# jhbastek/PhysicsInformedDiffusionModels

Hardware: AMD Instinct MI355X
Metric: training samples/sec (UNet+PDE-residual step), 64x64 Darcy (higher is better)
Workload: dtype f32

## Files before the change

### physicsinformeddiffusionmodels_amd/csrc/k_attn_proj.hip

```cpp
#include "pidm_launch.h"

namespace pidm {

static const int kLapDH = 32;
constexpr int kLapSmallNT = 1024;
static const int kLapTileLd = 33;

__device__ __forceinline__ float lap_exp(float x) { return __expf(x); }
__device__ __forceinline__ int lap_row(int r, int half) { return (r & 3) + 8 * (r >> 2) + 4 * half; }

static int lap_nper_div() {
  const char* e = knob("PIDM_LAP_NPER_DIV");
  const int v = e ? atoi(e) : 1;
  return (v == 2 || v == 4) ? v : 1;
}
static int lap_nper(int N, int C, int slabs) {
  int n = (slabs == 1 ? 512 : 256) * 32 / C;
  if (slabs == 3) n = (C == 32) ? 32 : n / 2;
  if (slabs == 2 && n / lap_nper_div() >= 64) n /= lap_nper_div();
  while (n > 32 && N % n) n >>= 1;
  return n;
}

template <int CB>
__global__ void __launch_bounds__(512) lap_kctx_kernel(const float* __restrict__ xn, const float* __restrict__ wqkv,
                                                       float* __restrict__ part, int N, int heads, int nper) {
  constexpr int C = 32 * CB, CP = C + 4;
  HIP_DYNAMIC_SHARED(float, smem)
  float* xs = smem;
  float* fs = smem + (size_t)nper * CP;
  const int tid = threadIdx.x, lane = tid & 63, half = lane >> 5, l31 = lane & 31;
  const int wave = __builtin_amdgcn_readfirstlane(tid >> 6);
  const int NS = N / nper;
  const int b = blockIdx.x / NS, ns = blockIdx.x % NS;
  const int HD = heads * kLapDH;
  const float* xb = xn + ((size_t)b * N + (size_t)ns * nper) * C;
  for (int e = tid; e < nper * (C / 4); e += 512) {
    const int px = e / (C / 4), q = e - px * (C / 4);
    *reinterpret_cast<f32x4*>(xs + (size_t)px * CP + 4 * q) = *reinterpret_cast<const f32x4*>(xb + (size_t)px * C + 4 * q);
  }
  __syncthreads();
  const int h = wave;
  if (h >= heads) return;
  f32x4 wk[C / 8];
  const float* wrow = wqkv + ((size_t)HD + h * kLapDH + l31) * C + 4 * half;
#pragma unroll
  for (int g8 = 0; g8 < C / 8; ++g8) wk[g8] = *reinterpret_cast<const f32x4*>(wrow + 8 * g8);
  f32x16 M[CB];
#pragma unroll
  for (int cb = 0; cb < CB; ++cb)
    for (int r = 0; r < 16; ++r) M[cb][r] = 0.f;
  float mrun = -3.0e38f, zp = 0.f;
  float* fw = fs + wave * 32;
  for (int t = 0; t < nper / 32; ++t) {
    f32x16 kt;
    for (int r = 0; r < 16; ++r) kt[r] = 0.f;
    const float* arow = xs + (size_t)(t * 32 + l31) * CP + 4 * half;
#pragma unroll
    for (int g8 = 0; g8 < C / 8; ++g8) {
      const f32x4 a4 = *reinterpret_cast<const f32x4*>(arow + 8 * g8);
#pragma unroll
      for (int s = 0; s < 4; ++s) kt = __builtin_amdgcn_mfma_f32_32x32x2f32(a4[s], wk[g8][s], kt, 0, 0, 0);
    }
    float tm = kt[0];
#pragma unroll
    for (int r = 1; r < 16; ++r) tm = fmaxf(tm, kt[r]);
    tm = fmaxf(tm, pidm_other_half(tm));
    if (__any(tm > mrun)) {
      const float mn = fmaxf(mrun, tm);
      const float f = lap_exp(mrun - mn);
      zp *= f;
      mrun = mn;
      if (half == 0) fw[l31] = f;
      PIDM_WAVE_LDS_SYNC();
#pragma unroll
      for (int q4 = 0; q4 < 4; ++q4) {
        const f32x4 f4 = *reinterpret_cast<const f32x4*>(fw + 8 * q4 + 4 * half);
#pragma unroll
        for (int cb = 0; cb < CB; ++cb)
#pragma unroll
          for (int i = 0; i < 4; ++i) M[cb][4 * q4 + i] *= f4[i];
      }
      PIDM_WAVE_LDS_SYNC();
    }
#pragma unroll
    for (int r = 0; r < 16; ++r) {
      kt[r] = lap_exp(kt[r] - mrun);
      zp += kt[r];
    }
#pragma unroll
    for (int r = 0; r < 16; ++r) {
      const float* brow = xs + (size_t)(t * 32 + lap_row(r, half)) * CP + l31;
#pragma unroll
      for (int cb = 0; cb < CB; ++cb) M[cb] = __builtin_amdgcn_mfma_f32_32x32x2f32(kt[r], brow[32 * cb], M[cb], 0, 0, 0);
    }
  }
  const float z = zp + pidm_other_half(zp);
  float* o = part + ((size_t)blockIdx.x * heads + h) * (size_t)(32 * C + 64);
#pragma unroll
  for (int cb = 0; cb < CB; ++cb)
#pragma unroll
    for (int r = 0; r < 16; ++r) o[(size_t)lap_row(r, half) * C + 32 * cb + l31] = M[cb][r];
  if (half == 0) {
    o[32 * C + l31] = mrun;
    o[32 * C + 32 + l31] = z;
  }
}

static int lap_nper_split(int N, int C) {
  int n = 256 * 32 / C;
  if (n / lap_nper_div() >= 64) n /= lap_nper_div();
  while (n > 32 && N % n) n >>= 1;
  return n;
}
static int lap_groups(int heads, int ntiles) {
  const char* e = knob("PIDM_LAP_GROUPS");
  int g = 8 / heads;
  if (e && atoi(e) > 0 && atoi(e) < g) g = atoi(e);
  while (g > 1 && ntiles % g) --g;
  return g < 1 ? 1 : g;
}
template <int CB>
__global__ void __launch_bounds__(512) lap_kctx_split_kernel(const float* __restrict__ xn, const float* __restrict__ wqkv,
                                                             float* __restrict__ part, int N, int heads, int nper) {
  constexpr int C = 32 * CB, RA = 6 * C + 16;
  HIP_DYNAMIC_SHARED(float, smemf)
  char* smem = reinterpret_cast<char*>(smemf);
  const int RT = nper * 2 + 16;
  char* XA = smem;
  char* XT = smem + (size_t)nper * RA;
  float* fs = reinterpret_cast<float*>(XT + (size_t)3 * C * RT);
  const int tid = threadIdx.x, lane = tid & 63, half = lane >> 5, l31 = lane & 31;
  const int wave = __builtin_amdgcn_readfirstlane(tid >> 6);
  const int NS = N / nper;
  const int b = blockIdx.x / NS, ns = blockIdx.x % NS;
  const int HD = heads * kLapDH;
  const float* xb = xn + ((size_t)b * N + (size_t)ns * nper) * C;
  {
    constexpr int QN = C / 4, GP = 16 / QN;
    const int q = lane & (QN - 1), pb = (lane & 15) / QN, la = lane >> 4;
    for (int sl = wave; sl < nper / (4 * GP); sl += 8) {
      const int px = (sl * GP + pb) * 4 + la;
      const f32x4 v = *reinterpret_cast<const f32x4*>(xb + (size_t)px * C + 4 * q);
      typedef unsigned u32x2_t __attribute__((ext_vector_type(2)));
      unsigned a0, a1, a2, b0, b1, b2;
      pidm_split3_pk(v[0], v[1], a0, a1, a2);
      pidm_split3_pk(v[2], v[3], b0, b1, b2);
      char* da = XA + (size_t)px * RA + 8 * q;
      *reinterpret_cast<u32x2_t*>(da) = u32x2_t{a0, b0};
      *reinterpret_cast<u32x2_t*>(da + 2 * C) = u32x2_t{a1, b1};
      *reinterpret_cast<u32x2_t*>(da + 4 * C) = u32x2_t{a2, b2};
      unsigned t0 = __float_as_uint(v[0]), t1 = __float_as_uint(v[1]), t2 = __float_as_uint(v[2]), t3 = __float_as_uint(v[3]);
      {
        const auto s02 = __builtin_amdgcn_permlane32_swap(t0, t2, false, false);
        const auto s13 = __builtin_amdgcn_permlane32_swap(t1, t3, false, false);
        const auto s01 = __builtin_amdgcn_permlane16_swap(s02[0], s13[0], false, false);
        const auto s23 = __builtin_amdgcn_permlane16_swap(s02[1], s13[1], false, false);
        t0 = s01[0]; t1 = s01[1]; t2 = s23[0]; t3 = s23[1];
      }
      pidm_split3_pk(__uint_as_float(t0), __uint_as_float(t1), a0, a1, a2);
      pidm_split3_pk(__uint_as_float(t2), __uint_as_float(t3), b0, b1, b2);
      char* dt = XT + (size_t)(4 * q + la) * RT + (size_t)((sl * GP + pb) * 4) * 2;
      *reinterpret_cast<u32x2_t*>(dt) = u32x2_t{a0, b0};
      *reinterpret_cast<u32x2_t*>(dt + (size_t)C * RT) = u32x2_t{a1, b1};
      *reinterpret_cast<u32x2_t*>(dt + (size_t)2 * C * RT) = u32x2_t{a2, b2};
    }
  }
  __syncthreads();
  const int h = wave;
  if (h >= heads) return;
  u32x4 wk[C / 16][3];
  {
    const float* wrow = wqkv + ((size_t)HD + h * kLapDH + l31) * C + 8 * half;
#pragma unroll
    for (int s = 0; s < C / 16; ++s) {
      const f32x4 w0 = *reinterpret_cast<const f32x4*>(wrow + 16 * s), w1 = *reinterpret_cast<const f32x4*>(wrow + 16 * s + 4);
      unsigned p0[4], p1[4], p2[4];
      pidm_split3_pk(w0[0], w0[1], p0[0], p1[0], p2[0]);
      pidm_split3_pk(w0[2], w0[3], p0[1], p1[1], p2[1]);
      pidm_split3_pk(w1[0], w1[1], p0[2], p1[2], p2[2]);
      pidm_split3_pk(w1[2], w1[3], p0[3], p1[3], p2[3]);
      wk[s][0] = u32x4{p0[0], p0[1], p0[2], p0[3]};
      wk[s][1] = u32x4{p1[0], p1[1], p1[2], p1[3]};
      wk[s][2] = u32x4{p2[0], p2[1], p2[2], p2[3]};
    }
  }
  f32x16 M[CB];
#pragma unroll
  for (int cb = 0; cb < CB; ++cb)
    for (int r = 0; r < 16; ++r) M[cb][r] = 0.f;
  float mrun = -3.0e38f, zp = 0.f;
  float* fw = fs + wave * 32;
#define PIDM_LAP_SIX(acc_, a_, b_)                                                                                 \
  acc_ = pidm_mfma_bf16_32x32x16(a_[2], b_[0], acc_);                                                              \
  acc_ = pidm_mfma_bf16_32x32x16(a_[0], b_[2], acc_);                                                              \
  acc_ = pidm_mfma_bf16_32x32x16(a_[1], b_[1], acc_);                                                              \
  acc_ = pidm_mfma_bf16_32x32x16(a_[1], b_[0], acc_);                                                              \
  acc_ = pidm_mfma_bf16_32x32x16(a_[0], b_[1], acc_);                                                              \
  acc_ = pidm_mfma_bf16_32x32x16(a_[0], b_[0], acc_);
  for (int t = 0; t < nper / 32; ++t) {
    f32x16 kt;
    for (int r = 0; r < 16; ++r) kt[r] = 0.f;
    const char* arow = XA + (size_t)(t * 32 + l31) * RA + 16 * half;
#pragma unroll
    for (int s = 0; s < C / 16; ++s) {
      u32x4 xa[3];
#pragma unroll
      for (int pc = 0; pc < 3; ++pc) xa[pc] = *reinterpret_cast<const u32x4*>(arow + pc * 2 * C + 32 * s);
      PIDM_LAP_SIX(kt, xa, wk[s])
    }
    float tm = kt[0];
#pragma unroll
    for (int r = 1; r < 16; ++r) tm = fmaxf(tm, kt[r]);
    tm = fmaxf(tm, pidm_other_half(tm));
    if (__any(tm > mrun)) {
      const float mn = fmaxf(mrun, tm);
      const float f = lap_exp(mrun - mn);
      zp *= f;
      mrun = mn;
      if (half == 0) fw[l31] = f;
      PIDM_WAVE_LDS_SYNC();
#pragma unroll
      for (int q4 = 0; q4 < 4; ++q4) {
        const f32x4 f4 = *reinterpret_cast<const f32x4*>(fw + 8 * q4 + 4 * half);
#pragma unroll
        for (int cb = 0; cb < CB; ++cb)
#pragma unroll
          for (int i = 0; i < 4; ++i) M[cb][4 * q4 + i] *= f4[i];
      }
      PIDM_WAVE_LDS_SYNC();
    }
#pragma unroll
    for (int r = 0; r < 16; ++r) {
      kt[r] = lap_exp(kt[r] - mrun);
      zp += kt[r];
    }
#pragma unroll
    for (int s = 0; s < 2; ++s) {
      u32x4 ea[3];
      {
        unsigned p0[4], p1[4], p2[4];
#pragma unroll
        for (int j = 0; j < 4; ++j) pidm_split3_pk(kt[8 * s + 2 * j], kt[8 * s + 2 * j + 1], p0[j], p1[j], p2[j]);
        ea[0] = u32x4{p0[0], p0[1], p0[2], p0[3]};
        ea[1] = u32x4{p1[0], p1[1], p1[2], p1[3]};
        ea[2] = u32x4{p2[0], p2[1], p2[2], p2[3]};
      }
#pragma unroll
      for (int cb = 0; cb < CB; ++cb) {
        u32x4 xb4[3];
        const char* brow = XT + (size_t)(32 * cb + l31) * RT + (size_t)(t * 32 + 16 * s + 4 * half) * 2;
#pragma unroll
        for (int pc = 0; pc < 3; ++pc) {
          typedef unsigned u32x2_t __attribute__((ext_vector_type(2)));
          const u32x2_t lo = *reinterpret_cast<const u32x2_t*>(brow + (size_t)pc * C * RT);
          const u32x2_t hi = *reinterpret_cast<const u32x2_t*>(brow + (size_t)pc * C * RT + 16);
          xb4[pc] = u32x4{lo[0], lo[1], hi[0], hi[1]};
        }
        PIDM_LAP_SIX(M[cb], ea, xb4)
      }
    }
  }
#undef PIDM_LAP_SIX
  const float z = zp + pidm_other_half(zp);
  float* o = part + ((size_t)blockIdx.x * heads + h) * (size_t)(32 * C + 64);
#pragma unroll
  for (int cb = 0; cb < CB; ++cb)
#pragma unroll
    for (int r = 0; r < 16; ++r) o[(size_t)lap_row(r, half) * C + 32 * cb + l31] = M[cb][r];
  if (half == 0) {
    o[32 * C + l31] = mrun;
    o[32 * C + 32 + l31] = z;
  }
}

__global__ void __launch_bounds__(kLapSmallNT) lap_kctx_final_kernel(const float* __restrict__ part, const float* __restrict__ wqkv,
                                                             const float* __restrict__ wout, float* __restrict__ kst,
                                                             float* __restrict__ Mmat, float* __restrict__ ctx,
                                                             float* __restrict__ P, int N, int heads, int C, int NS) {
  HIP_DYNAMIC_SHARED(float, smem)
  float* sM = smem;
  float* sW = sM + 32 * C;
  float* sC = sW + 32 * (C + 1) + C;
  float* sw = sC + 32 * 33;
  float* sst = sw + NS * 32;
  __shared__ float sm_[32], siz[32];
  constexpr int NT = kLapSmallNT;
  const int b = blockIdx.x / heads, h = blockIdx.x % heads, tid = threadIdx.x;
  const int HD = heads * kLapDH;
  const size_t pstride = (size_t)(32 * C + 64);
  const float* p0 = part + ((size_t)b * NS * heads + h) * pstride;
  for (int e = tid; e < NS * 64; e += NT) sst[e] = p0[(size_t)(e >> 6) * heads * pstride + 32 * C + (e & 63)];
  __syncthreads();
  if (tid < 32) {
    float m = -3.0e38f;
    for (int k = 0; k < NS; ++k) m = fmaxf(m, sst[k * 64 + tid]);
    float z = 0.f;
    for (int k = 0; k < NS; ++k) {
      const float w = lap_exp(sst[k * 64 + tid] - m);
      sw[k * 32 + tid] = w;
      z += sst[k * 64 + 32 + tid] * w;
    }
    sm_[tid] = m;
    siz[tid] = 1.f / z;
    kst[((size_t)blockIdx.x * 32 + tid) * 2] = m;
    kst[((size_t)blockIdx.x * 32 + tid) * 2 + 1] = 1.f / z;
  }
  __syncthreads();
  for (int e = tid; e < 32 * C; e += NT) {
    const int d = e / C;
    float v = 0.f;
    for (int k = 0; k < NS; ++k) v += p0[(size_t)k * heads * pstride + e] * sw[k * 32 + d];
    v *= siz[d];
    sM[e] = v;
    Mmat[(size_t)blockIdx.x * 32 * C + e] = v;
    const int c = e - d * C;
    sW[d * (C + 1) + c] = wqkv[((size_t)2 * HD + h * kLapDH + d) * C + c];
  }
  __syncthreads();
  const float invN = 1.f / (float)N;
  for (int e = tid; e < 1024; e += NT) {
    const int d = e >> 5, ee = e & 31;
    float v = 0.f;
    for (int c = 0; c < C; ++c) v = fmaf(sM[d * C + c], sW[ee * (C + 1) + c], v);
    v *= invN;
    sC[d * 33 + ee] = v;
    ctx[(size_t)blockIdx.x * 1024 + e] = v;
  }
  __syncthreads();
  for (int e = tid; e < 32 * C; e += NT) {
    const int cc = e >> 5, ee = e & 31;
    sW[cc * 33 + ee] = wout[(size_t)cc * HD + h * kLapDH + ee];
  }
  __syncthreads();
  for (int e = tid; e < 32 * C; e += NT) {
    const int d = e / C, cc = e - d * C;
    float v = 0.f;
#pragma unroll
    for (int ee = 0; ee < 32; ++ee) v = fmaf(sC[d * 33 + ee], sW[cc * 33 + ee], v);
    P[(size_t)blockIdx.x * 32 * C + e] = v;
  }
}

template <int CB>
__global__ void __launch_bounds__(256) lap_out_kernel(const float* __restrict__ xn, const float* __restrict__ wqkv,
                                                      const float* __restrict__ P, const float* __restrict__ bias,
                                                      const float* __restrict__ resid, float* __restrict__ y,
                                                      float* __restrict__ qstat, int N, int heads, int tiles_per_wg, float scale) {
  constexpr int C = 32 * CB, CP = C + 4;
  HIP_DYNAMIC_SHARED(float, smem)
  const int HD = heads * kLapDH;
  float* sWq = smem;
  float* sP = smem + (size_t)HD * CP;
  const int tid = threadIdx.x, lane = tid & 63, half = lane >> 5, l31 = lane & 31;
  const int wave = __builtin_amdgcn_readfirstlane(tid >> 6);
  const int wgs_per_img = (N / 32 + tiles_per_wg - 1) / tiles_per_wg;
  const int b = blockIdx.x / wgs_per_img, wg = blockIdx.x % wgs_per_img;
  for (int e = tid; e < HD * (C / 4); e += 256) {
    const int row = e / (C / 4), q = e - row * (C / 4);
    *reinterpret_cast<f32x4*>(sWq + (size_t)row * CP + 4 * q) = *reinterpret_cast<const f32x4*>(wqkv + (size_t)row * C + 4 * q);
    *reinterpret_cast<f32x4*>(sP + (size_t)row * C + 4 * q) = *reinterpret_cast<const f32x4*>(P + ((size_t)b * HD + row) * C + 4 * q);
  }
  __syncthreads();
  const int t_end = (wg + 1) * tiles_per_wg < N / 32 ? (wg + 1) * tiles_per_wg : N / 32;
  for (int t = wg * tiles_per_wg + wave; t < t_end; t += 4) {
    const size_t pix = (size_t)b * N + (size_t)t * 32 + l31;
    f32x4 xt[C / 8];
#pragma unroll
    for (int g8 = 0; g8 < C / 8; ++g8) xt[g8] = *reinterpret_cast<const f32x4*>(xn + pix * C + 8 * g8 + 4 * half);
    f32x16 yacc[CB];
#pragma unroll
    for (int cb = 0; cb < CB; ++cb)
      for (int r = 0; r < 16; ++r) yacc[cb][r] = 0.f;
    for (int h = 0; h < heads; ++h) {
      f32x16 qt;
      for (int r = 0; r < 16; ++r) qt[r] = 0.f;
      const float* wrow = sWq + (size_t)(h * kLapDH + l31) * CP + 4 * half;
#pragma unroll
      for (int g8 = 0; g8 < C / 8; ++g8) {
        const f32x4 w4 = *reinterpret_cast<const f32x4*>(wrow + 8 * g8);
#pragma unroll
        for (int s = 0; s < 4; ++s) qt = __builtin_amdgcn_mfma_f32_32x32x2f32(w4[s], xt[g8][s], qt, 0, 0, 0);
      }
      float mx = qt[0];
#pragma unroll
      for (int r = 1; r < 16; ++r) mx = fmaxf(mx, qt[r]);
      mx = fmaxf(mx, pidm_other_half(mx));
      float sm = 0.f;
#pragma unroll
      for (int r = 0; r < 16; ++r) {
        qt[r] = lap_exp(qt[r] - mx);
        sm += qt[r];
      }
      sm += pidm_other_half(sm);
      const float inv = 1.f / sm;
      if (half == 0) *reinterpret_cast<float2*>(qstat + (pix * heads + h) * 2) = make_float2(mx, inv);
      const float sc = inv * scale;
      const float* prow = sP + (size_t)(h * kLapDH) * C + l31;
#pragma unroll
      for (int r = 0; r < 16; ++r) {
        const float qv = qt[r] * sc;
        const float* pr = prow + (size_t)lap_row(r, half) * C;
#pragma unroll
        for (int cb = 0; cb < CB; ++cb) yacc[cb] = __builtin_amdgcn_mfma_f32_32x32x2f32(pr[32 * cb], qv, yacc[cb], 0, 0, 0);
      }
    }
#pragma unroll
    for (int cb = 0; cb < CB; ++cb)
#pragma unroll
      for (int q4 = 0; q4 < 4; ++q4) {
        const int c0 = 32 * cb + 8 * q4 + 4 * half;
        const f32x4 bv = *reinterpret_cast<const f32x4*>(bias + c0);
        const f32x4 rv = *reinterpret_cast<const f32x4*>(resid + pix * C + c0);
        f32x4 o;
#pragma unroll
        for (int i = 0; i < 4; ++i) o[i] = yacc[cb][4 * q4 + i] + bv[i] + rv[i];
        *reinterpret_cast<f32x4*>(y + pix * C + c0) = o;
      }
  }
}

__global__ void __launch_bounds__(512) lap_out_split_kernel(const float* __restrict__ xn, const float* __restrict__ wqkv,
                                                            const float* __restrict__ P, const float* __restrict__ bias,
                                                            const float* __restrict__ resid, float* __restrict__ y,
                                                            float* __restrict__ qstat, int N, int heads, int tiles_per_wg, float scale) {
  constexpr int C = 32, RA = 6 * C + 16;
  HIP_DYNAMIC_SHARED(float, smemf)
  char* smem = reinterpret_cast<char*>(smemf);
  const int HD = heads * kLapDH;
  const int RT = HD * 2 + 16;
  char* WA = smem;
  char* PT = smem + (size_t)HD * RA;
  const int tid = threadIdx.x, lane = tid & 63, half = lane >> 5, l31 = lane & 31;
  const int wave = __builtin_amdgcn_readfirstlane(tid >> 6);
  const int wgs_per_img = (N / 32 + tiles_per_wg - 1) / tiles_per_wg;
  const int b = blockIdx.x / wgs_per_img, wg = blockIdx.x % wgs_per_img;
  typedef unsigned u32x2_t __attribute__((ext_vector_type(2)));
  {
    const int q = lane & 7, pb = (lane >> 3) & 1, la = lane >> 4;
    for (int sl = wave; sl < HD / 8; sl += 8) {
      const int d = (sl * 2 + pb) * 4 + la;
      const f32x4 v = *reinterpret_cast<const f32x4*>(wqkv + (size_t)d * C + 4 * q);
      const f32x4 w = *reinterpret_cast<const f32x4*>(P + ((size_t)b * HD + d) * C + 4 * q);
      unsigned a0, a1, a2, b0, b1, b2;
      pidm_split3_pk(v[0], v[1], a0, a1, a2);
      pidm_split3_pk(v[2], v[3], b0, b1, b2);
      char* da = WA + (size_t)d * RA + 8 * q;
      *reinterpret_cast<u32x2_t*>(da) = u32x2_t{a0, b0};
      *reinterpret_cast<u32x2_t*>(da + 2 * C) = u32x2_t{a1, b1};
      *reinterpret_cast<u32x2_t*>(da + 4 * C) = u32x2_t{a2, b2};
      unsigned t0 = __float_as_uint(w[0]), t1 = __float_as_uint(w[1]), t2 = __float_as_uint(w[2]), t3 = __float_as_uint(w[3]);
      {
        const auto s02 = __builtin_amdgcn_permlane32_swap(t0, t2, false, false);
        const auto s13 = __builtin_amdgcn_permlane32_swap(t1, t3, false, false);
        const auto s01 = __builtin_amdgcn_permlane16_swap(s02[0], s13[0], false, false);
        const auto s23 = __builtin_amdgcn_permlane16_swap(s02[1], s13[1], false, false);
        t0 = s01[0]; t1 = s01[1]; t2 = s23[0]; t3 = s23[1];
      }
      pidm_split3_pk(__uint_as_float(t0), __uint_as_float(t1), a0, a1, a2);
      pidm_split3_pk(__uint_as_float(t2), __uint_as_float(t3), b0, b1, b2);
      char* dt = PT + (size_t)(4 * q + la) * RT + (size_t)((sl * 2 + pb) * 4) * 2;
      *reinterpret_cast<u32x2_t*>(dt) = u32x2_t{a0, b0};
      *reinterpret_cast<u32x2_t*>(dt + (size_t)C * RT) = u32x2_t{a1, b1};
      *reinterpret_cast<u32x2_t*>(dt + (size_t)2 * C * RT) = u32x2_t{a2, b2};
    }
  }
  __syncthreads();
#define PIDM_LAP_SIX(acc_, a_, b_)                                                                                 \
  acc_ = pidm_mfma_bf16_32x32x16(a_[2], b_[0], acc_);                                                              \
  acc_ = pidm_mfma_bf16_32x32x16(a_[0], b_[2], acc_);                                                              \
  acc_ = pidm_mfma_bf16_32x32x16(a_[1], b_[1], acc_);                                                              \
  acc_ = pidm_mfma_bf16_32x32x16(a_[1], b_[0], acc_);                                                              \
  acc_ = pidm_mfma_bf16_32x32x16(a_[0], b_[1], acc_);                                                              \
  acc_ = pidm_mfma_bf16_32x32x16(a_[0], b_[0], acc_);
  const int t_end = (wg + 1) * tiles_per_wg < N / 32 ? (wg + 1) * tiles_per_wg : N / 32;
  for (int t = wg * tiles_per_wg + wave; t < t_end; t += 8) {
    const size_t pix = (size_t)b * N + (size_t)t * 32 + l31;
    u32x4 xb[C / 16][3];
#pragma unroll
    for (int s = 0; s < C / 16; ++s) {
      const f32x4 x0 = *reinterpret_cast<const f32x4*>(xn + pix * C + 16 * s + 8 * half);
      const f32x4 x1 = *reinterpret_cast<const f32x4*>(xn + pix * C + 16 * s + 8 * half + 4);
      unsigned p0[4], p1[4], p2[4];
      pidm_split3_pk(x0[0], x0[1], p0[0], p1[0], p2[0]);
      pidm_split3_pk(x0[2], x0[3], p0[1], p1[1], p2[1]);
      pidm_split3_pk(x1[0], x1[1], p0[2], p1[2], p2[2]);
      pidm_split3_pk(x1[2], x1[3], p0[3], p1[3], p2[3]);
      xb[s][0] = u32x4{p0[0], p0[1], p0[2], p0[3]};
      xb[s][1] = u32x4{p1[0], p1[1], p1[2], p1[3]};
      xb[s][2] = u32x4{p2[0], p2[1], p2[2], p2[3]};
    }
    f32x16 yacc;
    for (int r = 0; r < 16; ++r) yacc[r] = 0.f;
    for (int h = 0; h < heads; ++h) {
      f32x16 qt;
      for (int r = 0; r < 16; ++r) qt[r] = 0.f;
      const char* wrow = WA + (size_t)(h * kLapDH + l31) * RA + 16 * half;
#pragma unroll
      for (int s = 0; s < C / 16; ++s) {
        u32x4 wa[3];
#pragma unroll
        for (int pc = 0; pc < 3; ++pc) wa[pc] = *reinterpret_cast<const u32x4*>(wrow + pc * 2 * C + 32 * s);
        PIDM_LAP_SIX(qt, wa, xb[s])
      }
      float mx = qt[0];
#pragma unroll
      for (int r = 1; r < 16; ++r) mx = fmaxf(mx, qt[r]);
      mx = fmaxf(mx, pidm_other_half(mx));
      float sm = 0.f;
#pragma unroll
      for (int r = 0; r < 16; ++r) {
        qt[r] = lap_exp(qt[r] - mx);
        sm += qt[r];
      }
      sm += pidm_other_half(sm);
      const float inv = 1.f / sm;
      if (half == 0) *reinterpret_cast<float2*>(qstat + (pix * heads + h) * 2) = make_float2(mx, inv);
      const float sc = inv * scale;
#pragma unroll
      for (int s = 0; s < 2; ++s) {
        u32x4 qb[3], pa[3];
        {
          unsigned p0[4], p1[4], p2[4];
#pragma unroll
          for (int j = 0; j < 4; ++j) pidm_split3_pk(qt[8 * s + 2 * j] * sc, qt[8 * s + 2 * j + 1] * sc, p0[j], p1[j], p2[j]);
          qb[0] = u32x4{p0[0], p0[1], p0[2], p0[3]};
          qb[1] = u32x4{p1[0], p1[1], p1[2], p1[3]};
          qb[2] = u32x4{p2[0], p2[1], p2[2], p2[3]};
        }
        const char* prow = PT + (size_t)l31 * RT + (size_t)(h * kLapDH + 16 * s + 4 * half) * 2;
#pragma unroll
        for (int pc = 0; pc < 3; ++pc) {
          const u32x2_t lo = *reinterpret_cast<const u32x2_t*>(prow + (size_t)pc * C * RT);
          const u32x2_t hi = *reinterpret_cast<const u32x2_t*>(prow + (size_t)pc * C * RT + 16);
          pa[pc] = u32x4{lo[0], lo[1], hi[0], hi[1]};
        }
        PIDM_LAP_SIX(yacc, pa, qb)
      }
    }
#pragma unroll
    for (int q4 = 0; q4 < 4; ++q4) {
      const int c0 = 8 * q4 + 4 * half;
      const f32x4 bv = *reinterpret_cast<const f32x4*>(bias + c0);
      const f32x4 rv = *reinterpret_cast<const f32x4*>(resid + pix * C + c0);
      f32x4 o;
#pragma unroll
      for (int i = 0; i < 4; ++i) o[i] = yacc[4 * q4 + i] + bv[i] + rv[i];
      *reinterpret_cast<f32x4*>(y + pix * C + c0) = o;
    }
  }
#undef PIDM_LAP_SIX
}

template <int CB>
__global__ void __launch_bounds__(512) lap_g_kernel(const float* __restrict__ xn, const float* __restrict__ dy,
                                                    const float* __restrict__ wqkv, const float* __restrict__ qstat,
                                                    float* __restrict__ part, int N, int heads, int nper, float scale) {
  constexpr int C = 32 * CB, CP = C + 4;
  HIP_DYNAMIC_SHARED(float, smem)
  float* xs = smem;
  float* ys = smem + (size_t)nper * CP;
  const int tid = threadIdx.x, lane = tid & 63, half = lane >> 5, l31 = lane & 31;
  const int wave = __builtin_amdgcn_readfirstlane(tid >> 6);
  const int NS = N / nper;
  const int b = blockIdx.x / NS, ns = blockIdx.x % NS;
  const size_t pix0 = (size_t)b * N + (size_t)ns * nper;
  for (int e = tid; e < nper * (C / 4); e += 512) {
    const int px = e / (C / 4), q = e - px * (C / 4);
    *reinterpret_cast<f32x4*>(xs + (size_t)px * CP + 4 * q) = *reinterpret_cast<const f32x4*>(xn + (pix0 + px) * C + 4 * q);
    *reinterpret_cast<f32x4*>(ys + (size_t)px * CP + 4 * q) = *reinterpret_cast<const f32x4*>(dy + (pix0 + px) * C + 4 * q);
  }
  __syncthreads();
  const int h = wave;
  if (h >= heads) return;
  f32x4 wq[C / 8];
  const float* wrow = wqkv + ((size_t)h * kLapDH + l31) * C + 4 * half;
#pragma unroll
  for (int g8 = 0; g8 < C / 8; ++g8) wq[g8] = *reinterpret_cast<const f32x4*>(wrow + 8 * g8);
  f32x16 G[CB];
#pragma unroll
  for (int cb = 0; cb < CB; ++cb)
    for (int r = 0; r < 16; ++r) G[cb][r] = 0.f;
  for (int t = 0; t < nper / 32; ++t) {
    f32x16 qt;
    for (int r = 0; r < 16; ++r) qt[r] = 0.f;
    const float* arow = xs + (size_t)(t * 32 + l31) * CP + 4 * half;
#pragma unroll
    for (int g8 = 0; g8 < C / 8; ++g8) {
      const f32x4 a4 = *reinterpret_cast<const f32x4*>(arow + 8 * g8);
#pragma unroll
      for (int s = 0; s < 4; ++s) qt = __builtin_amdgcn_mfma_f32_32x32x2f32(a4[s], wq[g8][s], qt, 0, 0, 0);
    }
    const float* st = qstat + ((pix0 + (size_t)t * 32) * heads + h) * 2;
#pragma unroll
    for (int r = 0; r < 16; ++r) {
      const int px = lap_row(r, half);
      const float2 s2 = *reinterpret_cast<const float2*>(st + (size_t)px * heads * 2);
      const float qv = lap_exp(qt[r] - s2.x) * s2.y * scale;
      const float* brow = ys + (size_t)(t * 32 + px) * CP + l31;
#pragma unroll
      for (int cb = 0; cb < CB; ++cb) G[cb] = __builtin_amdgcn_mfma_f32_32x32x2f32(qv, brow[32 * cb], G[cb], 0, 0, 0);
    }
  }
  float* o = part + ((size_t)blockIdx.x * heads + h) * (size_t)(32 * C);
#pragma unroll
  for (int cb = 0; cb < CB; ++cb)
#pragma unroll
    for (int r = 0; r < 16; ++r) o[(size_t)lap_row(r, half) * C + 32 * cb + l31] = G[cb][r];
}

template <int CB>
__global__ void __launch_bounds__(512) lap_g_split_kernel(const float* __restrict__ xn, const float* __restrict__ dy,
                                                          const float* __restrict__ wqkv, const float* __restrict__ qstat,
                                                          float* __restrict__ part, int N, int heads, int nper, float scale) {
  constexpr int C = 32 * CB, RA = 6 * C + 16;
  HIP_DYNAMIC_SHARED(float, smemf)
  char* smem = reinterpret_cast<char*>(smemf);
  const int RT = nper * 2 + 16;
  char* XA = smem;
  char* YT = smem + (size_t)nper * RA;
  const int tid = threadIdx.x, lane = tid & 63, half = lane >> 5, l31 = lane & 31;
  const int wave = __builtin_amdgcn_readfirstlane(tid >> 6);
  const int NS = N / nper;
  const int b = blockIdx.x / NS, ns = blockIdx.x % NS;
  const size_t pix0 = (size_t)b * N + (size_t)ns * nper;
  {
    constexpr int QN = C / 4, GP = 16 / QN;
    const int q = lane & (QN - 1), pb = (lane & 15) / QN, la = lane >> 4;
    typedef unsigned u32x2_t __attribute__((ext_vector_type(2)));
    for (int sl = wave; sl < nper / (4 * GP); sl += 8) {
      const int px = (sl * GP + pb) * 4 + la;
      const f32x4 v = *reinterpret_cast<const f32x4*>(xn + (pix0 + px) * C + 4 * q);
      const f32x4 w = *reinterpret_cast<const f32x4*>(dy + (pix0 + px) * C + 4 * q);
      unsigned a0, a1, a2, b0, b1, b2;
      pidm_split3_pk(v[0], v[1], a0, a1, a2);
      pidm_split3_pk(v[2], v[3], b0, b1, b2);
      char* da = XA + (size_t)px * RA + 8 * q;
      *reinterpret_cast<u32x2_t*>(da) = u32x2_t{a0, b0};
      *reinterpret_cast<u32x2_t*>(da + 2 * C) = u32x2_t{a1, b1};
      *reinterpret_cast<u32x2_t*>(da + 4 * C) = u32x2_t{a2, b2};
      unsigned t0 = __float_as_uint(w[0]), t1 = __float_as_uint(w[1]), t2 = __float_as_uint(w[2]), t3 = __float_as_uint(w[3]);
      {
        const auto s02 = __builtin_amdgcn_permlane32_swap(t0, t2, false, false);
        const auto s13 = __builtin_amdgcn_permlane32_swap(t1, t3, false, false);
        const auto s01 = __builtin_amdgcn_permlane16_swap(s02[0], s13[0], false, false);
        const auto s23 = __builtin_amdgcn_permlane16_swap(s02[1], s13[1], false, false);
        t0 = s01[0]; t1 = s01[1]; t2 = s23[0]; t3 = s23[1];
      }
      pidm_split3_pk(__uint_as_float(t0), __uint_as_float(t1), a0, a1, a2);
      pidm_split3_pk(__uint_as_float(t2), __uint_as_float(t3), b0, b1, b2);
      char* dt = YT + (size_t)(4 * q + la) * RT + (size_t)((sl * GP + pb) * 4) * 2;
      *reinterpret_cast<u32x2_t*>(dt) = u32x2_t{a0, b0};
      *reinterpret_cast<u32x2_t*>(dt + (size_t)C * RT) = u32x2_t{a1, b1};
      *reinterpret_cast<u32x2_t*>(dt + (size_t)2 * C * RT) = u32x2_t{a2, b2};
    }
  }
  __syncthreads();
  const int h = wave;
  if (h >= heads) return;
  u32x4 wq[C / 16][3];
  {
    const float* wrow = wqkv + ((size_t)h * kLapDH + l31) * C + 8 * half;
#pragma unroll
    for (int s = 0; s < C / 16; ++s) {
      const f32x4 w0 = *reinterpret_cast<const f32x4*>(wrow + 16 * s), w1 = *reinterpret_cast<const f32x4*>(wrow + 16 * s + 4);
      unsigned p0[4], p1[4], p2[4];
      pidm_split3_pk(w0[0], w0[1], p0[0], p1[0], p2[0]);
      pidm_split3_pk(w0[2], w0[3], p0[1], p1[1], p2[1]);
      pidm_split3_pk(w1[0], w1[1], p0[2], p1[2], p2[2]);
      pidm_split3_pk(w1[2], w1[3], p0[3], p1[3], p2[3]);
      wq[s][0] = u32x4{p0[0], p0[1], p0[2], p0[3]};
      wq[s][1] = u32x4{p1[0], p1[1], p1[2], p1[3]};
      wq[s][2] = u32x4{p2[0], p2[1], p2[2], p2[3]};
    }
  }
  f32x16 G[CB];
#pragma unroll
  for (int cb = 0; cb < CB; ++cb)
    for (int r = 0; r < 16; ++r) G[cb][r] = 0.f;
#define PIDM_LAP_SIX(acc_, a_, b_)                                                                                 \
  acc_ = pidm_mfma_bf16_32x32x16(a_[2], b_[0], acc_);                                                              \
  acc_ = pidm_mfma_bf16_32x32x16(a_[0], b_[2], acc_);                                                              \
  acc_ = pidm_mfma_bf16_32x32x16(a_[1], b_[1], acc_);                                                              \
  acc_ = pidm_mfma_bf16_32x32x16(a_[1], b_[0], acc_);                                                              \
  acc_ = pidm_mfma_bf16_32x32x16(a_[0], b_[1], acc_);                                                              \
  acc_ = pidm_mfma_bf16_32x32x16(a_[0], b_[0], acc_);
  for (int t = 0; t < nper / 32; ++t) {
    f32x16 qt;
    for (int r = 0; r < 16; ++r) qt[r] = 0.f;
    const char* arow = XA + (size_t)(t * 32 + l31) * RA + 16 * half;
#pragma unroll
    for (int s = 0; s < C / 16; ++s) {
      u32x4 xa[3];
#pragma unroll
      for (int pc = 0; pc < 3; ++pc) xa[pc] = *reinterpret_cast<const u32x4*>(arow + pc * 2 * C + 32 * s);
      PIDM_LAP_SIX(qt, xa, wq[s])
    }
    const float* st = qstat + ((pix0 + (size_t)t * 32) * heads + h) * 2;
#pragma unroll
    for (int r = 0; r < 16; ++r) {
      const float2 s2 = *reinterpret_cast<const float2*>(st + (size_t)lap_row(r, half) * heads * 2);
      qt[r] = lap_exp(qt[r] - s2.x) * s2.y * scale;
    }
#pragma unroll
    for (int s = 0; s < 2; ++s) {
      u32x4 ea[3];
      {
        unsigned p0[4], p1[4], p2[4];
#pragma unroll
        for (int j = 0; j < 4; ++j) pidm_split3_pk(qt[8 * s + 2 * j], qt[8 * s + 2 * j + 1], p0[j], p1[j], p2[j]);
        ea[0] = u32x4{p0[0], p0[1], p0[2], p0[3]};
        ea[1] = u32x4{p1[0], p1[1], p1[2], p1[3]};
        ea[2] = u32x4{p2[0], p2[1], p2[2], p2[3]};
      }
#pragma unroll
      for (int cb = 0; cb < CB; ++cb) {
        u32x4 yb4[3];
        const char* brow = YT + (size_t)(32 * cb + l31) * RT + (size_t)(t * 32 + 16 * s + 4 * half) * 2;
#pragma unroll
        for (int pc = 0; pc < 3; ++pc) {
          typedef unsigned u32x2_t __attribute__((ext_vector_type(2)));
          const u32x2_t lo = *reinterpret_cast<const u32x2_t*>(brow + (size_t)pc * C * RT);
          const u32x2_t hi = *reinterpret_cast<const u32x2_t*>(brow + (size_t)pc * C * RT + 16);
          yb4[pc] = u32x4{lo[0], lo[1], hi[0], hi[1]};
        }
        PIDM_LAP_SIX(G[cb], ea, yb4)
      }
    }
  }
#undef PIDM_LAP_SIX
  float* o = part + ((size_t)blockIdx.x * heads + h) * (size_t)(32 * C);
#pragma unroll
  for (int cb = 0; cb < CB; ++cb)
#pragma unroll
    for (int r = 0; r < 16; ++r) o[(size_t)lap_row(r, half) * C + 32 * cb + l31] = G[cb][r];
}

__global__ void __launch_bounds__(kLapSmallNT) lap_mid_kernel(const float* __restrict__ gpart, const float* __restrict__ wqkv,
                                                      const float* __restrict__ wout, const float* __restrict__ ctx,
                                                      const float* __restrict__ Mmat, float* __restrict__ dMmat,
                                                      float* __restrict__ rowdot, float* __restrict__ dwout_part,
                                                      float* __restrict__ dwv_part, int N, int heads, int C, int NS) {
  HIP_DYNAMIC_SHARED(float, smem)
  float* sG = smem;
  float* sW = sG + 32 * (C + 1);
  float* sD = sW + (C > 33 ? C : 33) * 33 + 32 * (C + 1);
  float* sM = sD + 32 * 33;
  constexpr int NT = kLapSmallNT;
  const int b = blockIdx.x / heads, h = blockIdx.x % heads, tid = threadIdx.x;
  const int HD = heads * kLapDH;
  const float* g0 = gpart + ((size_t)b * NS * heads + h) * (size_t)(32 * C);
  for (int e = tid; e < 32 * C; e += NT) {
    const int d = e / C, c = e - d * C;
    float v = 0.f;
    for (int k0 = 0; k0 < NS; k0 += 8) {
      float t[8];
#pragma unroll
      for (int u = 0; u < 8; ++u) t[u] = g0[(size_t)(k0 + u < NS ? k0 + u : 0) * heads * 32 * C + e];
#pragma unroll
      for (int u = 0; u < 8; ++u) v += (k0 + u < NS) ? t[u] : 0.f;
    }
    sG[d * (C + 1) + c] = v;
    sM[d * (C + 1) + c] = Mmat[(size_t)blockIdx.x * 32 * C + e];
    const int cc = e >> 5, ee = e & 31;
    sW[cc * 33 + ee] = wout[(size_t)cc * HD + h * kLapDH + ee];
  }
  __syncthreads();
  for (int e = tid; e < 1024; e += NT) {
    const int d = e >> 5, ee = e & 31;
    float v = 0.f;
    for (int c = 0; c < C; ++c) v = fmaf(sG[d * (C + 1) + c], sW[c * 33 + ee], v);
    sD[d * 33 + ee] = v;
  }
  for (int e = tid; e < 32 * C; e += NT) {
    const int cc = e >> 5, ee = e & 31;
    float v = 0.f;
#pragma unroll 8
    for (int d = 0; d < 32; ++d) v = fmaf(sG[d * (C + 1) + cc], ctx[(size_t)blockIdx.x * 1024 + d * 32 + ee], v);
    dwout_part[((size_t)b * C + cc) * HD + h * kLapDH + ee] = v;
  }
  __syncthreads();
  for (int e = tid; e < 32 * C; e += NT) {
    const int ee = e / C, c = e - ee * C;
    sW[ee * (C + 1) + c] = wqkv[((size_t)2 * HD + h * kLapDH + ee) * C + c];
  }
  __syncthreads();
  const float invN = 1.f / (float)N;
  for (int e = tid; e < 32 * C; e += NT) {
    const int ee = e / C, c = e - ee * C;
    float v = 0.f;
#pragma unroll 8
    for (int d = 0; d < 32; ++d) v = fmaf(sD[d * 33 + ee], sM[d * (C + 1) + c], v);
    dwv_part[((size_t)b * HD + h * kLapDH + ee) * C + c] = v * invN;
  }
  __syncthreads();
  for (int e = tid; e < 32 * C; e += NT) {
    const int d = e / C, c = e - d * C;
    float v = 0.f;
#pragma unroll 8
    for (int ee = 0; ee < 32; ++ee) v = fmaf(sD[d * 33 + ee], sW[ee * (C + 1) + c], v);
    v *= invN;
    dMmat[(size_t)blockIdx.x * 32 * C + e] = v;
    sG[d * (C + 1) + c] = v * sM[d * (C + 1) + c];
  }
  __syncthreads();
  if (tid < 32) {
    float v = 0.f;
    for (int c = 0; c < C; ++c) v += sG[tid * (C + 1) + c];
    rowdot[(size_t)blockIdx.x * 32 + tid] = v;
  }
}

#ifndef PIDM_LAP_TRACE_BUILD
#define PIDM_LAP_TRACE_BUILD 0
#endif
__device__ unsigned long long g_lap_trace[2 * 8 * 16];
template <int CB, bool SP>
__global__ void __launch_bounds__(512) lap_bwd_kernel(const float* __restrict__ xn, const float* __restrict__ dy,
                                                      const float* __restrict__ wqkv, const float* __restrict__ P,
                                                      const float* __restrict__ kst, const float* __restrict__ dMmat,
                                                      const float* __restrict__ rowdot, float* __restrict__ dxn,
                                                      float* __restrict__ dw_part, int N, int heads, int nper, int nsub,
                                                      float scale, int split_dw, int G) {
  constexpr int C = 32 * CB, CP = C + 4;
  static_assert(!SP || CB == 1, "the split projections keep the head's operand matrices in registers: C = 32 only");
  constexpr int WCP = SP ? C : CP;
  constexpr int PR = 208;
  HIP_DYNAMIC_SHARED(float, smem)
  float* xs = smem;
  float* ys = xs + (SP ? 0 : (size_t)nper * CP);
  constexpr int TSZ = CB * 32 * kLapTileLd;
  float* tiles = ys + (SP ? 0 : (size_t)nper * CP);
  float* cst = tiles + (size_t)8 * TSZ;
  constexpr bool WLDS = (CB == 1);
  float* wl = cst + 8 * 96;
  const int RT = nper * 2 + (WLDS ? 0 : 16);
  const int HD = heads * kLapDH;
  char* XT = reinterpret_cast<char*>(wl + (WLDS ? 3 * HD * WCP : 0));
  char* XP = XT + (size_t)3 * C * RT;
  char* YP = XP + (size_t)nper * PR;
  const int tid = threadIdx.x, lane = tid & 63, half = lane >> 5, l31 = lane & 31;
  const int wave = __builtin_amdgcn_readfirstlane(tid >> 6);
  const int NW = N / (nper * nsub);
  const int b = blockIdx.x / NW, nw = blockIdx.x % NW;
  if (WLDS) {
    for (int e = tid; e < 3 * HD * (C / 4); e += 512) {
      const int m = e / (HD * (C / 4)), rem = e - m * (HD * (C / 4));
      const int row = rem / (C / 4), q = rem - row * (C / 4);
      const float* src = (m < 2) ? wqkv + ((size_t)m * HD + row) * C : dMmat + ((size_t)b * HD + row) * C;
      *reinterpret_cast<f32x4*>(wl + ((size_t)m * HD + row) * WCP + 4 * q) = *reinterpret_cast<const f32x4*>(src + 4 * q);
    }
  }
  const int tg = wave / heads, h = wave - tg * heads;
  const bool act = tg < G;
  float* tw = tiles + (size_t)wave * TSZ;
  float* cw = cst + wave * 96;
  if (act && half == 0) {
    cw[l31] = kst[(((size_t)b * heads + h) * 32 + l31) * 2];
    cw[32 + l31] = kst[(((size_t)b * heads + h) * 32 + l31) * 2 + 1];
    cw[64 + l31] = rowdot[((size_t)b * heads + h) * 32 + l31];
  }
  f32x16 dWq[CB], dWk[CB];
  const size_t bh = (size_t)b * heads + (act ? h : 0);
  const int hrow = (act ? h : 0) * kLapDH + l31;
  const float* wq_p = WLDS ? wl + (size_t)hrow * WCP + 4 * half : wqkv + (size_t)hrow * C + 4 * half;
  const float* wk_p = WLDS ? wl + (size_t)(HD + hrow) * WCP + 4 * half : wqkv + ((size_t)HD + hrow) * C + 4 * half;
  const float* dm_p = WLDS ? wl + (size_t)(2 * HD + hrow) * WCP + 4 * half : dMmat + (bh * 32 + l31) * C + 4 * half;
  const float* pp_p = P + (bh * 32 + l31) * C + 4 * half;
  u32x4 fwq[SP ? C / 16 : 1][3], fwk[SP ? C / 16 : 1][3], fpp[SP ? C / 16 : 1][3], fdm[SP ? C / 16 : 1][3];
  if constexpr (SP) {
    __syncthreads();
#pragma unroll
    for (int ks = 0; ks < C / 16; ++ks) {
      const float* srcs[4] = {wl + (size_t)hrow * WCP + 16 * ks + 8 * half, wl + (size_t)(HD + hrow) * WCP + 16 * ks + 8 * half,
                              P + (bh * 32 + l31) * C + 16 * ks + 8 * half, wl + (size_t)(2 * HD + hrow) * WCP + 16 * ks + 8 * half};
#pragma unroll
      for (int m = 0; m < 4; ++m) {
        const f32x4 v0 = *reinterpret_cast<const f32x4*>(srcs[m]), v1 = *reinterpret_cast<const f32x4*>(srcs[m] + 4);
        unsigned q0[4], q1[4], q2[4];
        pidm_split3_pk(v0[0], v0[1], q0[0], q1[0], q2[0]);
        pidm_split3_pk(v0[2], v0[3], q0[1], q1[1], q2[1]);
        pidm_split3_pk(v1[0], v1[1], q0[2], q1[2], q2[2]);
        pidm_split3_pk(v1[2], v1[3], q0[3], q1[3], q2[3]);
        u32x4(&f)[3] = (m == 0) ? fwq[ks] : (m == 1) ? fwk[ks] : (m == 2) ? fpp[ks] : fdm[ks];
        f[0] = u32x4{q0[0], q0[1], q0[2], q0[3]};
        f[1] = u32x4{q1[0], q1[1], q1[2], q1[3]};
        f[2] = u32x4{q2[0], q2[1], q2[2], q2[3]};
      }
    }
  }
  if (act) {
#pragma unroll
    for (int cb = 0; cb < CB; ++cb)
      for (int r = 0; r < 16; ++r) { dWq[cb][r] = 0.f; dWk[cb][r] = 0.f; }
  }
  const int ldT = WLDS ? WCP : C;
  const int hT = act ? h : 0;
  const float* wqT = WLDS ? wl + (size_t)(hT * kLapDH) * WCP + l31 : wqkv + (size_t)hT * kLapDH * C + l31;
  const float* wkT = WLDS ? wl + (size_t)(HD + hT * kLapDH) * WCP + l31 : wqkv + ((size_t)HD + hT * kLapDH) * C + l31;
  const float* dmT = WLDS ? wl + (size_t)(2 * HD + hT * kLapDH) * WCP + l31 : dMmat + ((size_t)b * heads + hT) * 32 * C + l31;

  const float rscale = 1.f / scale;
#define PIDM_LAP_DW(g_, dW_)                                                                                       \
  if (split_dw) {                                                                                                  \
    _Pragma("unroll") for (int r = 0; r < 16; ++r) tw[lap_row(r, half) * kLapTileLd + l31] = g_[r];                \
    PIDM_WAVE_LDS_SYNC();                                                                                          \
    _Pragma("unroll") for (int s = 0; s < 2; ++s) {                                                                \
      float g0[4], g1[4];                                                                                          \
      _Pragma("unroll") for (int e = 0; e < 4; ++e) {                                                              \
        g0[e] = tw[l31 * kLapTileLd + 16 * s + 8 * half + e];                                                      \
        g1[e] = tw[l31 * kLapTileLd + 16 * s + 8 * half + 4 + e];                                                  \
      }                                                                                                            \
      unsigned p0[4], p1[4], p2[4];                                                                                \
      pidm_split3_pk(g0[0], g0[1], p0[0], p1[0], p2[0]);                                                           \
      pidm_split3_pk(g0[2], g0[3], p0[1], p1[1], p2[1]);                                                           \
      pidm_split3_pk(g1[0], g1[1], p0[2], p1[2], p2[2]);                                                           \
      pidm_split3_pk(g1[2], g1[3], p0[3], p1[3], p2[3]);                                                           \
      u32x4 ga[3] = {u32x4{p0[0], p0[1], p0[2], p0[3]}, u32x4{p1[0], p1[1], p1[2], p1[3]}, u32x4{p2[0], p2[1], p2[2], p2[3]}}; \
      _Pragma("unroll") for (int cb = 0; cb < CB; ++cb) {                                                          \
        u32x4 xb4[3];                                                                                              \
        const char* brow = XT + (size_t)(32 * cb + l31) * RT + (size_t)(t * 32 + 16 * s + 8 * half) * 2;           \
        _Pragma("unroll") for (int pc = 0; pc < 3; ++pc) xb4[pc] = *reinterpret_cast<const u32x4*>(brow + (size_t)pc * C * RT); \
        dW_[cb] = pidm_mfma_bf16_32x32x16(ga[2], xb4[0], dW_[cb]);                                                 \
        dW_[cb] = pidm_mfma_bf16_32x32x16(ga[0], xb4[2], dW_[cb]);                                                 \
        dW_[cb] = pidm_mfma_bf16_32x32x16(ga[1], xb4[1], dW_[cb]);                                                 \
        dW_[cb] = pidm_mfma_bf16_32x32x16(ga[1], xb4[0], dW_[cb]);                                                 \
        dW_[cb] = pidm_mfma_bf16_32x32x16(ga[0], xb4[1], dW_[cb]);                                                 \
        dW_[cb] = pidm_mfma_bf16_32x32x16(ga[0], xb4[0], dW_[cb]);                                                 \
      }                                                                                                            \
    }                                                                                                              \
    PIDM_WAVE_LDS_SYNC();                                                                                          \
  } else {                                                                                                         \
    _Pragma("unroll") for (int r = 0; r < 16; ++r) tw[lap_row(r, half) * kLapTileLd + l31] = g_[r];                \
    PIDM_WAVE_LDS_SYNC();                                                                                          \
    _Pragma("unroll") for (int s = 0; s < 16; ++s) {                                                               \
      const float a = tw[l31 * kLapTileLd + 2 * s + half];                                                         \
      const float* brow = xs + (size_t)(t * 32 + 2 * s + half) * CP + l31;                                         \
      _Pragma("unroll") for (int cb = 0; cb < CB; ++cb) dW_[cb] = __builtin_amdgcn_mfma_f32_32x32x2f32(a, brow[32 * cb], dW_[cb], 0, 0, 0); \
    }                                                                                                              \
    PIDM_WAVE_LDS_SYNC();                                                                                          \
  }
#define PIDM_LAP_SIX(acc_, fa_, fb_)                                                                               \
  acc_ = pidm_mfma_bf16_32x32x16(fa_[2], fb_[0], acc_);                                                            \
  acc_ = pidm_mfma_bf16_32x32x16(fa_[0], fb_[2], acc_);                                                            \
  acc_ = pidm_mfma_bf16_32x32x16(fa_[1], fb_[1], acc_);                                                            \
  acc_ = pidm_mfma_bf16_32x32x16(fa_[1], fb_[0], acc_);                                                            \
  acc_ = pidm_mfma_bf16_32x32x16(fa_[0], fb_[1], acc_);                                                            \
  acc_ = pidm_mfma_bf16_32x32x16(fa_[0], fb_[0], acc_);
  const bool order_flip = (split_dw & 2) != 0;
  if ((split_dw & 8) && wave >= 4) __builtin_amdgcn_s_setprio(1);
#if PIDM_LAP_TRACE_BUILD
  const bool tr_on = (split_dw & 4) && blockIdx.x == 0 && (wave & 3) == 0;
  int tr_round = 0;
#define PIDM_LAP_STAMP(i_)                                                                                         \
  if (tr_on && tr_round < 8) {                                                                                     \
    const unsigned long long c__ = clock64();                                                                      \
    if (lane == 0) g_lap_trace[(wave >> 2) * 128 + 16 * tr_round + (i_)] = c__;                                    \
  }
#define PIDM_LAP_TRACE_ONLY(x_) x_
#else
#define PIDM_LAP_STAMP(i_)
#define PIDM_LAP_TRACE_ONLY(x_)
#endif
  split_dw &= 1;
  const bool k_first = (wave & 4) != 0 && order_flip;
  for (int sub = 0; sub < nsub; ++sub) {
  const size_t pix0 = (size_t)b * N + ((size_t)nw * nsub + sub) * nper;
  for (int e = tid; e < nper * (C / 4); e += 512) {
    const int px = e / (C / 4), q = e - px * (C / 4);
    const f32x4 vx = *reinterpret_cast<const f32x4*>(xn + (pix0 + px) * C + 4 * q);
    const f32x4 vy = *reinterpret_cast<const f32x4*>(dy + (pix0 + px) * C + 4 * q);
    if constexpr (SP) {
      typedef unsigned u32x2_t __attribute__((ext_vector_type(2)));
      const size_t o = (size_t)px * PR + ((q >> 2) * 2 + ((q >> 1) & 1)) * 48 + (q & 1) * 8;
      unsigned a0, a1, a2, b0, b1, b2;
      pidm_split3_pk(vx[0], vx[1], a0, a1, a2);
      pidm_split3_pk(vx[2], vx[3], b0, b1, b2);
      *reinterpret_cast<u32x2_t*>(XP + o) = u32x2_t{a0, b0};
      *reinterpret_cast<u32x2_t*>(XP + o + 16) = u32x2_t{a1, b1};
      *reinterpret_cast<u32x2_t*>(XP + o + 32) = u32x2_t{a2, b2};
      pidm_split3_pk(vy[0], vy[1], a0, a1, a2);
      pidm_split3_pk(vy[2], vy[3], b0, b1, b2);
      *reinterpret_cast<u32x2_t*>(YP + o) = u32x2_t{a0, b0};
      *reinterpret_cast<u32x2_t*>(YP + o + 16) = u32x2_t{a1, b1};
      *reinterpret_cast<u32x2_t*>(YP + o + 32) = u32x2_t{a2, b2};
    } else {
      *reinterpret_cast<f32x4*>(xs + (size_t)px * CP + 4 * q) = vx;
      *reinterpret_cast<f32x4*>(ys + (size_t)px * CP + 4 * q) = vy;
    }
  }
  if (split_dw) {
    constexpr int QN = C / 4, GP = 16 / QN;
    const int q = lane & (QN - 1), pb = (lane & 15) / QN, la = lane >> 4;
    typedef unsigned u32x2_t __attribute__((ext_vector_type(2)));
    for (int sl = wave; sl < nper / (4 * GP); sl += 8) {
      const int px = (sl * GP + pb) * 4 + la;
      const f32x4 w = *reinterpret_cast<const f32x4*>(xn + (pix0 + px) * C + 4 * q);
      unsigned t0 = __float_as_uint(w[0]), t1 = __float_as_uint(w[1]), t2 = __float_as_uint(w[2]), t3 = __float_as_uint(w[3]);
      {
        const auto s02 = __builtin_amdgcn_permlane32_swap(t0, t2, false, false);
        const auto s13 = __builtin_amdgcn_permlane32_swap(t1, t3, false, false);
        const auto s01 = __builtin_amdgcn_permlane16_swap(s02[0], s13[0], false, false);
        const auto s23 = __builtin_amdgcn_permlane16_swap(s02[1], s13[1], false, false);
        t0 = s01[0]; t1 = s01[1]; t2 = s23[0]; t3 = s23[1];
      }
      unsigned a0, a1, a2, b0, b1, b2;
      pidm_split3_pk(__uint_as_float(t0), __uint_as_float(t1), a0, a1, a2);
      pidm_split3_pk(__uint_as_float(t2), __uint_as_float(t3), b0, b1, b2);
      char* dt = XT + (size_t)(4 * q + la) * RT + (size_t)((sl * GP + pb) * 4) * 2;
      *reinterpret_cast<u32x2_t*>(dt) = u32x2_t{a0, b0};
      *reinterpret_cast<u32x2_t*>(dt + (size_t)C * RT) = u32x2_t{a1, b1};
      *reinterpret_cast<u32x2_t*>(dt + (size_t)2 * C * RT) = u32x2_t{a2, b2};
    }
  }
  __syncthreads();
  for (int t0 = 0; t0 < nper / 32; t0 += G) {
    const int t = t0 + tg;
    f32x16 dx[CB];
    PIDM_LAP_STAMP(0)
    PIDM_LAP_TRACE_ONLY(int tr_half = 0;)
    if (act) {
      int z0 = 0;
      if (!WLDS) PIDM_OPAQUE_I32(z0);
#pragma unroll
      for (int cb = 0; cb < CB; ++cb)
        for (int r = 0; r < 16; ++r) dx[cb][r] = 0.f;
      const float* xrow = xs + (size_t)(t * 32 + l31) * CP + 4 * half;
      const float* yrow = ys + (size_t)(t * 32 + l31) * CP + 4 * half;
      const char* xpr = XP + (size_t)(t * 32 + l31) * PR + 48 * half;
      const char* ypr = YP + (size_t)(t * 32 + l31) * PR + 48 * half;
      auto q_part = [&]() __attribute__((always_inline)) {
      f32x16 qt, dq;
      for (int r = 0; r < 16; ++r) { qt[r] = 0.f; dq[r] = 0.f; }
      if constexpr (SP) {
#pragma unroll
        for (int ks = 0; ks < C / 16; ++ks) {
          u32x4 xb[3], yb[3];
#pragma unroll
          for (int pc = 0; pc < 3; ++pc) {
            xb[pc] = *reinterpret_cast<const u32x4*>(xpr + 96 * ks + 16 * pc);
            yb[pc] = *reinterpret_cast<const u32x4*>(ypr + 96 * ks + 16 * pc);
          }
          PIDM_LAP_SIX(qt, fwq[ks], xb)
          PIDM_LAP_SIX(dq, fpp[ks], yb)
        }
      } else {
#pragma unroll 2
      for (int g8 = 0; g8 < C / 8; ++g8) {
        const f32x4 w4 = *reinterpret_cast<const f32x4*>(wq_p + z0 + 8 * g8);
        const f32x4 p4 = *reinterpret_cast<const f32x4*>(pp_p + z0 + 8 * g8);
        const f32x4 x4 = *reinterpret_cast<const f32x4*>(xrow + 8 * g8);
        const f32x4 y4 = *reinterpret_cast<const f32x4*>(yrow + 8 * g8);
#pragma unroll
        for (int s = 0; s < 4; ++s) {
          qt = __builtin_amdgcn_mfma_f32_32x32x2f32(w4[s], x4[s], qt, 0, 0, 0);
          dq = __builtin_amdgcn_mfma_f32_32x32x2f32(p4[s], y4[s], dq, 0, 0, 0);
        }
      }
      }
      float mx = qt[0];
#pragma unroll
      for (int r = 1; r < 16; ++r) mx = fmaxf(mx, qt[r]);
      mx = fmaxf(mx, pidm_other_half(mx));
      float sm = 0.f;
#pragma unroll
      for (int r = 0; r < 16; ++r) {
        qt[r] = lap_exp(qt[r] - mx);
        sm += qt[r];
      }
      sm += pidm_other_half(sm);
      const float sc = scale / sm;
      float jd = 0.f;
#pragma unroll
      for (int r = 0; r < 16; ++r) {
        qt[r] *= sc;
        jd += qt[r] * dq[r];
      }
      jd = (jd + pidm_other_half(jd)) * rscale;
#pragma unroll
      for (int r = 0; r < 16; ++r) dq[r] = qt[r] * (dq[r] - jd);
      PIDM_LAP_STAMP(1 + 3 * tr_half)
      if constexpr (WLDS) {
        float wa[16][CB];
#pragma unroll
        for (int r = 0; r < 16; ++r)
#pragma unroll
          for (int cb = 0; cb < CB; ++cb) wa[r][cb] = (wqT + (size_t)lap_row(r, half) * ldT)[32 * cb];
#pragma unroll
        for (int r = 0; r < 16; ++r)
#pragma unroll
          for (int cb = 0; cb < CB; ++cb) dx[cb] = __builtin_amdgcn_mfma_f32_32x32x2f32(wa[r][cb], dq[r], dx[cb], 0, 0, 0);
      } else {
#pragma unroll
        for (int r = 0; r < 16; ++r) {
          const float* wr = wqT + (size_t)lap_row(r, half) * ldT;
#pragma unroll
          for (int cb = 0; cb < CB; ++cb) dx[cb] = __builtin_amdgcn_mfma_f32_32x32x2f32(wr[32 * cb], dq[r], dx[cb], 0, 0, 0);
        }
      }
      PIDM_LAP_STAMP(2 + 3 * tr_half)
      PIDM_LAP_DW(dq, dWq)
      PIDM_LAP_STAMP(3 + 3 * tr_half)
      PIDM_LAP_TRACE_ONLY(tr_half = 1;)
      };
      auto k_part = [&]() __attribute__((always_inline)) {
      f32x16 kt, dk;
      for (int r = 0; r < 16; ++r) { kt[r] = 0.f; dk[r] = 0.f; }
      if constexpr (SP) {
#pragma unroll
        for (int ks = 0; ks < C / 16; ++ks) {
          u32x4 xb[3];
#pragma unroll
          for (int pc = 0; pc < 3; ++pc) xb[pc] = *reinterpret_cast<const u32x4*>(xpr + 96 * ks + 16 * pc);
          PIDM_LAP_SIX(kt, fwk[ks], xb)
          PIDM_LAP_SIX(dk, fdm[ks], xb)
        }
      } else {
#pragma unroll 2
      for (int g8 = 0; g8 < C / 8; ++g8) {
        const f32x4 w4 = *reinterpret_cast<const f32x4*>(wk_p + z0 + 8 * g8);
        const f32x4 m4 = *reinterpret_cast<const f32x4*>(dm_p + z0 + 8 * g8);
        const f32x4 x4 = *reinterpret_cast<const f32x4*>(xrow + 8 * g8);
#pragma unroll
        for (int s = 0; s < 4; ++s) {
          kt = __builtin_amdgcn_mfma_f32_32x32x2f32(w4[s], x4[s], kt, 0, 0, 0);
          dk = __builtin_amdgcn_mfma_f32_32x32x2f32(m4[s], x4[s], dk, 0, 0, 0);
        }
      }
      }
#pragma unroll
      for (int q4 = 0; q4 < 4; ++q4) {
        const f32x4 mx4 = *reinterpret_cast<const f32x4*>(cw + 8 * q4 + 4 * half);
        const f32x4 iz4 = *reinterpret_cast<const f32x4*>(cw + 32 + 8 * q4 + 4 * half);
        const f32x4 rd4 = *reinterpret_cast<const f32x4*>(cw + 64 + 8 * q4 + 4 * half);
#pragma unroll
        for (int i = 0; i < 4; ++i) {
          const int r = 4 * q4 + i;
          kt[r] = lap_exp(kt[r] - mx4[i]) * iz4[i];
          dk[r] = kt[r] * (dk[r] - rd4[i]);
        }
      }
      PIDM_LAP_STAMP(1 + 3 * tr_half)
      if constexpr (WLDS) {
        float wa[16][CB], ma[16][CB];
#pragma unroll
        for (int r = 0; r < 16; ++r)
#pragma unroll
          for (int cb = 0; cb < CB; ++cb) {
            wa[r][cb] = (wkT + (size_t)lap_row(r, half) * ldT)[32 * cb];
            ma[r][cb] = (dmT + (size_t)lap_row(r, half) * ldT)[32 * cb];
          }
#pragma unroll
        for (int r = 0; r < 16; ++r)
#pragma unroll
          for (int cb = 0; cb < CB; ++cb) {
            dx[cb] = __builtin_amdgcn_mfma_f32_32x32x2f32(wa[r][cb], dk[r], dx[cb], 0, 0, 0);
            dx[cb] = __builtin_amdgcn_mfma_f32_32x32x2f32(ma[r][cb], kt[r], dx[cb], 0, 0, 0);
          }
      } else {
#pragma unroll
        for (int r = 0; r < 16; ++r) {
          const float* wr = wkT + (size_t)lap_row(r, half) * ldT;
          const float* mr = dmT + (size_t)lap_row(r, half) * ldT;
#pragma unroll
          for (int cb = 0; cb < CB; ++cb) {
            dx[cb] = __builtin_amdgcn_mfma_f32_32x32x2f32(wr[32 * cb], dk[r], dx[cb], 0, 0, 0);
            dx[cb] = __builtin_amdgcn_mfma_f32_32x32x2f32(mr[32 * cb], kt[r], dx[cb], 0, 0, 0);
          }
        }
      }
      PIDM_LAP_STAMP(2 + 3 * tr_half)
      PIDM_LAP_DW(dk, dWk)
      PIDM_LAP_STAMP(3 + 3 * tr_half)
      PIDM_LAP_TRACE_ONLY(tr_half = 1;)
      };
      if (k_first) { k_part(); q_part(); } else { q_part(); k_part(); }
#pragma unroll
      for (int cb = 0; cb < CB; ++cb)
#pragma unroll
        for (int r = 0; r < 16; ++r) tw[(cb * 32 + lap_row(r, half)) * kLapTileLd + l31] = dx[cb][r];
    }
    PIDM_LAP_STAMP(7)
    __syncthreads();
    PIDM_LAP_STAMP(8)
    for (int e = tid; e < G * 32 * (C / 4); e += 512) {
      const int px = e / (C / 4), c0 = 4 * (e - px * (C / 4));
      const int gq = px >> 5, p31 = px & 31;
      f32x4 o = {0.f, 0.f, 0.f, 0.f};
      for (int w = gq * heads; w < (gq + 1) * heads; ++w) {
        const float* tp = tiles + (size_t)w * TSZ + (size_t)c0 * kLapTileLd + p31;
#pragma unroll
        for (int i = 0; i < 4; ++i) o[i] += tp[i * kLapTileLd];
      }
      *reinterpret_cast<f32x4*>(dxn + (pix0 + (size_t)t0 * 32 + px) * C + c0) = o;
    }
    PIDM_LAP_STAMP(9)
    __syncthreads();
    PIDM_LAP_STAMP(10)
    PIDM_LAP_TRACE_ONLY(++tr_round;)
  }
  }
#undef PIDM_LAP_STAMP
#undef PIDM_LAP_TRACE_ONLY
  for (int m = 0; m < 2 && G > 1; ++m) {
    if (act && tg > 0) {
#pragma unroll
      for (int cb = 0; cb < CB; ++cb)
#pragma unroll
        for (int r = 0; r < 16; ++r) tw[(cb * 32 + lap_row(r, half)) * kLapTileLd + l31] = m ? dWk[cb][r] : dWq[cb][r];
    }
    __syncthreads();
    if (act && tg == 0) {
      for (int g = 1; g < G; ++g) {
        const float* og = tiles + (size_t)(g * heads + h) * TSZ;
#pragma unroll
        for (int cb = 0; cb < CB; ++cb)
#pragma unroll
          for (int r = 0; r < 16; ++r) {
            const float v = og[(cb * 32 + lap_row(r, half)) * kLapTileLd + l31];
            if (m) dWk[cb][r] += v; else dWq[cb][r] += v;
          }
      }
    }
    __syncthreads();
  }
  if (act && tg == 0) {
    float* oq = dw_part + ((size_t)blockIdx.x * 2 * HD + h * kLapDH) * C;
    float* ok = oq + (size_t)HD * C;
#pragma unroll
    for (int cb = 0; cb < CB; ++cb)
#pragma unroll
      for (int r = 0; r < 16; ++r) {
        oq[(size_t)lap_row(r, half) * C + 32 * cb + l31] = dWq[cb][r];
        ok[(size_t)lap_row(r, half) * C + 32 * cb + l31] = dWk[cb][r];
      }
  }
#undef PIDM_LAP_DW
#undef PIDM_LAP_SIX
}

bool lap_ok(int N, int heads, int C, int Cout) {
  return Cout == C && (C == 32 || C == 64) && N % 32 == 0 && N >= 32 && heads >= 1 && heads <= 8;
}

size_t lap_scratch_floats(int B, int N, int heads, int C) {
  const size_t fw = (size_t)B * (N / lap_nper_split(N, C)) * heads * (32 * C + 64);
  const size_t bw = (size_t)B * (N / lap_nper(N, C, 2)) * heads * 32 * C;
  return (fw > bw ? fw : bw) + 64;
}
size_t lap_saved_floats(int B, int heads, int C) { return (size_t)B * heads * (64 + 32 * C + 1024 + 32 * C); }
static int lap_nsub(int N, int C) {
  const int ns = N / lap_nper(N, C, 3);
  int k = 1;
  while (k < 16 && ns % (2 * k) == 0 && ns / (2 * k) >= 8) k *= 2;
  return k;
}
size_t lap_dw_ranges(int N, int C) { return (size_t)(N / lap_nper(N, C, 3) / lap_nsub(N, C)); }

template <int CB>
static int lap_forward_t(const float* xn, const float* wqkv, const float* wout, const float* bias, const float* resid, float* y,
                         float* saved, float* qstat, int B, int N, int heads, float* scratch, hipStream_t st) {
  constexpr int C = 32 * CB;
  const char* spe = knob("PIDM_LAP_SPLIT");
  const bool split1 = !(spe && !atoi(spe));
  const int nper = split1 ? lap_nper_split(N, C) : lap_nper(N, C, 1), NS = N / nper;
  float* kst = saved;
  float* Mmat = kst + (size_t)B * heads * 64;
  float* ctx = Mmat + (size_t)B * heads * 32 * C;
  float* P = ctx + (size_t)B * heads * 1024;
  const size_t lds1 = ((size_t)nper * (C + 4) + 8 * 32) * sizeof(float);
  static bool attr = false;
  if (!attr) {
    (void)hipFuncSetAttribute(reinterpret_cast<const void*>(&lap_kctx_kernel<CB>), hipFuncAttributeMaxDynamicSharedMemorySize, 160 * 1024 - 256);
    (void)hipFuncSetAttribute(reinterpret_cast<const void*>(&lap_out_kernel<CB>), hipFuncAttributeMaxDynamicSharedMemorySize, 160 * 1024 - 256);
    (void)hipFuncSetAttribute(reinterpret_cast<const void*>(&lap_kctx_final_kernel), hipFuncAttributeMaxDynamicSharedMemorySize, 96 * 1024);
    attr = true;
  }
  if (split1) {
    const size_t ldss = (size_t)nper * (6 * C + 16) + (size_t)3 * C * (nper * 2 + 16) + 8 * 32 * sizeof(float);
    static bool attr_s = false;
    if (!attr_s) {
      (void)hipFuncSetAttribute(reinterpret_cast<const void*>(&lap_kctx_split_kernel<CB>), hipFuncAttributeMaxDynamicSharedMemorySize, 160 * 1024 - 256);
      attr_s = true;
    }
    PIDM_PROF_NAME("lap_kctx_split_kernel");
    hipLaunchKernelGGL(HIP_KERNEL_NAME(lap_kctx_split_kernel<CB>), dim3(B * NS), dim3(512), ldss, st, xn, wqkv, scratch, N, heads, nper);
  } else {
    hipLaunchKernelGGL(HIP_KERNEL_NAME(lap_kctx_kernel<CB>), dim3(B * NS), dim3(512), lds1, st, xn, wqkv, scratch, N, heads, nper);
  }
  PIDM_CHECK_LAUNCH("lap_kctx_kernel");
  const size_t lds2 = ((size_t)32 * C + 32 * (C + 1) + C + 32 * 33 + (size_t)NS * 96 + 64) * sizeof(float);
  hipLaunchKernelGGL(lap_kctx_final_kernel, dim3(B * heads), dim3(kLapSmallNT), lds2, st, scratch, wqkv, wout, kst, Mmat, ctx, P, N, heads, C, NS);
  PIDM_CHECK_LAUNCH("lap_kctx_final_kernel");
  const int HD = heads * kLapDH;
  const size_t lds3 = ((size_t)HD * (C + 4) + (size_t)HD * C) * sizeof(float);
  int tpw = 4;
  while ((long)B * ((N / 32 + tpw - 1) / tpw) > 2048 && tpw < 64) tpw *= 2;
  const int wgs = B * ((N / 32 + tpw - 1) / tpw);
  if (split1 && CB == 1 && HD % 8 == 0) {
    int tp8 = 8;
    while ((long)B * ((N / 32 + tp8 - 1) / tp8) > 1024 && tp8 < 64) tp8 *= 2;
    const int wg8 = B * ((N / 32 + tp8 - 1) / tp8);
    const size_t ldso = (size_t)HD * (6 * C + 16) + (size_t)3 * C * (HD * 2 + 16);
    static bool attr_o = false;
    if (!attr_o) {
      (void)hipFuncSetAttribute(reinterpret_cast<const void*>(&lap_out_split_kernel), hipFuncAttributeMaxDynamicSharedMemorySize, 160 * 1024 - 256);
      attr_o = true;
    }
    PIDM_PROF_NAME("lap_out_split_kernel");
    hipLaunchKernelGGL(lap_out_split_kernel, dim3(wg8), dim3(512), ldso, st, xn, wqkv, P, bias, resid, y, qstat, N, heads, tp8, 0.17677669529663687f);
  } else {
    hipLaunchKernelGGL(HIP_KERNEL_NAME(lap_out_kernel<CB>), dim3(wgs), dim3(256), lds3, st, xn, wqkv, P, bias, resid, y, qstat, N, heads, tpw,
                       0.17677669529663687f);
  }
  PIDM_CHECK_LAUNCH("lap_out_kernel");
  return 0;
}

int launch_lap_forward(const float* xn, const float* wqkv, const float* wout, const float* bias, const float* resid, float* y,
                       float* saved, float* qstat, int C, int B, int N, int heads, float* scratch, hipStream_t st) {
  if (!lap_ok(N, heads, C, C)) return fail("projected linear attention: unsupported shape (N=%d heads=%d C=%d)", N, heads, C);
  if (!bias || !resid) return fail("projected linear attention: bias and residual are required");
  if (C == 32) return lap_forward_t<1>(xn, wqkv, wout, bias, resid, y, saved, qstat, B, N, heads, scratch, st);
  return lap_forward_t<2>(xn, wqkv, wout, bias, resid, y, saved, qstat, B, N, heads, scratch, st);
}

template <int CB>
static int lap_backward_t(const float* xn, const float* dy, const float* wqkv, const float* wout, const float* saved, const float* qstat,
                          float* dxn, float* dwqk_part, float* dwv_part, float* dwout_part, float* tmp, int B, int N, int heads,
                          float* scratch, hipStream_t st) {
  constexpr int C = 32 * CB;
  const float scale = 0.17677669529663687f;
  const float* kst = saved;
  const float* Mmat = kst + (size_t)B * heads * 64;
  const float* ctx = Mmat + (size_t)B * heads * 32 * C;
  const float* P = ctx + (size_t)B * heads * 1024;
  float* dMmat = tmp;
  float* rowdot = tmp + (size_t)B * heads * 32 * C;
  static bool attr = false;
  if (!attr) {
    (void)hipFuncSetAttribute(reinterpret_cast<const void*>(&lap_g_kernel<CB>), hipFuncAttributeMaxDynamicSharedMemorySize, 160 * 1024 - 256);
    (void)hipFuncSetAttribute(reinterpret_cast<const void*>(&lap_bwd_kernel<CB, false>), hipFuncAttributeMaxDynamicSharedMemorySize, 160 * 1024 - 256);
    (void)hipFuncSetAttribute(reinterpret_cast<const void*>(&lap_mid_kernel), hipFuncAttributeMaxDynamicSharedMemorySize, 96 * 1024);
    attr = true;
  }
  const int np2 = lap_nper(N, C, 2), NS2 = N / np2;
  const size_t lds1 = (size_t)2 * np2 * (C + 4) * sizeof(float);
  const char* spe = knob("PIDM_LAP_SPLIT");
  if (!(spe && !atoi(spe))) {
    const size_t ldss = (size_t)np2 * (6 * C + 16) + (size_t)3 * C * (np2 * 2 + 16);
    static bool attr_s = false;
    if (!attr_s) {
      (void)hipFuncSetAttribute(reinterpret_cast<const void*>(&lap_g_split_kernel<CB>), hipFuncAttributeMaxDynamicSharedMemorySize, 160 * 1024 - 256);
      attr_s = true;
    }
    PIDM_PROF_NAME("lap_g_split_kernel");
    hipLaunchKernelGGL(HIP_KERNEL_NAME(lap_g_split_kernel<CB>), dim3(B * NS2), dim3(512), ldss, st, xn, dy, wqkv, qstat, scratch, N, heads, np2, scale);
  } else {
    hipLaunchKernelGGL(HIP_KERNEL_NAME(lap_g_kernel<CB>), dim3(B * NS2), dim3(512), lds1, st, xn, dy, wqkv, qstat, scratch, N, heads, np2, scale);
  }
  PIDM_CHECK_LAUNCH("lap_g_kernel");
  const size_t lds2 = ((size_t)32 * (C + 1) + (size_t)(C > 33 ? C : 33) * 33 + 32 * (C + 1) + 32 * 33 + 32 * (C + 1) + 64) * sizeof(float);
  hipLaunchKernelGGL(lap_mid_kernel, dim3(B * heads), dim3(kLapSmallNT), lds2, st, scratch, wqkv, wout, ctx, Mmat, dMmat, rowdot, dwout_part, dwv_part, N,
                     heads, C, NS2);
  PIDM_CHECK_LAUNCH("lap_mid_kernel");
  const int np3 = lap_nper(N, C, 3), nsub = lap_nsub(N, C), NS3 = N / np3 / nsub;
  int G3 = lap_groups(heads, 2), nslab = np3, nsl = nsub;
  if (G3 > 1 && (np3 / 32) % G3) {
    if (nsub % G3 == 0) { nslab = np3 * G3; nsl = nsub / G3; } else G3 = 1;
  }
  const char* ofe = knob("PIDM_LAP_ORDER_FLIP");
  const int oflip = (ofe && !atoi(ofe)) ? 0 : 2;
  const int split_dw = !(spe && !atoi(spe)) ? 1 : 0;
  const char* pre = knob("PIDM_LAP_PRIO");
  const int trbit = (knob("PIDM_LAP_TRACE") ? 4 : 0) | ((pre && atoi(pre)) ? 8 : 0);
  const char* ppe = knob("PIDM_LAP_SPLIT_PROJ");
  if (CB == 1 && split_dw && !(ppe && !atoi(ppe))) {
    const size_t lds3p = ((size_t)8 * 32 * kLapTileLd + 8 * 96 + (size_t)3 * heads * kLapDH * C) * sizeof(float) + (size_t)3 * C * (nslab * 2) +
                         (size_t)2 * nslab * 208;
    if (lds3p > 160 * 1024 - 256) return fail("lap_bwd: %zu B of LDS", lds3p);
    static bool attr_p = false;
    if (!attr_p) {
      (void)hipFuncSetAttribute(reinterpret_cast<const void*>(&lap_bwd_kernel<1, true>), hipFuncAttributeMaxDynamicSharedMemorySize, 160 * 1024 - 256);
      attr_p = true;
    }
    PIDM_PROF_NAME("lap_bwd_kernel<1, true>");
    hipLaunchKernelGGL(HIP_KERNEL_NAME(lap_bwd_kernel<1, true>), dim3(B * NS3), dim3(512), lds3p, st, xn, dy, wqkv, P, kst, dMmat, rowdot, dxn,
                       dwqk_part, N, heads, nslab, nsl, scale, 1 | oflip | trbit, G3);
    PIDM_CHECK_LAUNCH("lap_bwd_kernel");
    return 0;
  }
  const size_t lds3 = ((size_t)2 * nslab * (C + 4) + (size_t)8 * CB * 32 * kLapTileLd + 8 * 96 + (CB == 1 ? 3 * heads * kLapDH * (C + 4) : 0)) * sizeof(float) +
                      (size_t)3 * C * (nslab * 2 + (CB == 1 ? 0 : 16));
  if (lds3 > 160 * 1024 - 256) return fail("lap_bwd: %zu B of LDS", lds3);
  hipLaunchKernelGGL(HIP_KERNEL_NAME(lap_bwd_kernel<CB, false>), dim3(B * NS3), dim3(512), lds3, st, xn, dy, wqkv, P, kst, dMmat, rowdot, dxn, dwqk_part,
                     N, heads, nslab, nsl, scale, split_dw | oflip | trbit, G3);
  PIDM_CHECK_LAUNCH("lap_bwd_kernel");
  return 0;
}

size_t lap_bwd_tmp_floats(int B, int heads, int C) { return (size_t)B * heads * (32 * C + 32) + 64; }

int launch_lap_backward(const float* xn, const float* dy, const float* wqkv, const float* wout, const float* saved, const float* qstat,
                        float* dxn, float* dwqk_part, float* dwv_part, float* dwout_part, float* tmp, int C, int B, int N, int heads,
                        float* scratch, hipStream_t st) {
  if (!lap_ok(N, heads, C, C)) return fail("projected linear attention: unsupported shape (N=%d heads=%d C=%d)", N, heads, C);
  if (C == 32)
    return lap_backward_t<1>(xn, dy, wqkv, wout, saved, qstat, dxn, dwqk_part, dwv_part, dwout_part, tmp, B, N, heads, scratch, st);
  return lap_backward_t<2>(xn, dy, wqkv, wout, saved, qstat, dxn, dwqk_part, dwv_part, dwout_part, tmp, B, N, heads, scratch, st);
}

}

using namespace pidm;

extern "C" size_t pidm_lap_ws(int B, int N, int heads, int C) {
  const size_t HD = (size_t)heads * kLapDH;
  return (lap_scratch_floats(B, N, heads, C) + lap_bwd_tmp_floats(B, heads, C) + (size_t)B * lap_dw_ranges(N, C) * 2 * HD * C +
          (size_t)B * HD * C * 2 + 256) * sizeof(float);
}
extern "C" size_t pidm_lap_saved_floats(int B, int heads, int C) { return lap_saved_floats(B, heads, C); }

extern "C" int pidm_lap_forward(const float* xn, const float* w_qkv, const float* w_out, const float* bias, const float* resid, float* y,
                                float* saved, float* qstat, int C, int B, int N, int heads, void* workspace, void* stream) {
  if (!xn || !w_qkv || !w_out || !y || !saved || !qstat || !workspace) return fail("lap_forward: null buffer");
  return launch_lap_forward(xn, w_qkv, w_out, bias, resid, y, saved, qstat, C, B, N, heads, reinterpret_cast<float*>(workspace), as_stream(stream));
}

extern "C" int pidm_lap_backward(const float* xn, const float* dy, const float* w_qkv, const float* w_out, const float* saved,
                                 const float* qstat, float* d_xn, float* d_w_qkv, float* d_w_out, int C, int B, int N, int heads,
                                 void* workspace, void* stream) {
  if (!xn || !dy || !w_qkv || !w_out || !saved || !qstat || !d_xn || !d_w_qkv || !d_w_out || !workspace) return fail("lap_backward: null buffer");
  if (!lap_ok(N, heads, C, C)) return fail("projected linear attention: unsupported shape (N=%d heads=%d C=%d)", N, heads, C);
  hipStream_t st = as_stream(stream);
  const int HD = heads * kLapDH;
  float* scratch = reinterpret_cast<float*>(workspace);
  float* tmp = scratch + lap_scratch_floats(B, N, heads, C);
  float* dwqk = tmp + lap_bwd_tmp_floats(B, heads, C);
  const int nr = (int)lap_dw_ranges(N, C);
  float* dwv = dwqk + (size_t)B * nr * 2 * HD * C;
  float* dwo = dwv + (size_t)B * HD * C;
  if (launch_lap_backward(xn, dy, w_qkv, w_out, saved, qstat, d_xn, dwqk, dwv, dwo, tmp, C, B, N, heads, scratch, st)) return -1;
  if (launch_split_reduce(dwqk, d_w_qkv, nullptr, nullptr, B * nr, 2 * HD, C, 1, 2 * HD, C, st)) return -1;
  if (launch_split_reduce(dwv, d_w_qkv + (size_t)2 * HD * C, nullptr, nullptr, B, HD, C, 1, HD, C, st)) return -1;
  return launch_split_reduce(dwo, d_w_out, nullptr, nullptr, B, C, HD, 1, C, HD, st);
}

extern "C" int pidm_debug_lap_trace(unsigned long long* out256) {
  return hipMemcpyFromSymbol(out256, HIP_SYMBOL(pidm::g_lap_trace), sizeof(unsigned long long) * 256) == hipSuccess ? 0 : -1;
}
```

Before: 8194.

## Software-pipeline attention projection kernels to overlap MFMA with exp and loads

Adds a PIPE template variant, on by default, to the kctx-split, out-split and g-split linear-attention kernels. Global loads of weights and rows are issued early, before the staging barrier, so their latency overlaps with the LDS staging. The next tile's score MFMAs are interleaved with the current tile's exp and bf16-split VALU work using sched_barriers, and per-pixel q statistics are staged in LDS. This hides load and exp latency behind matrix-core work, at the cost of more registers, extra LDS and possible occupancy or spill pressure.

Result: no change. 8225, median of 6 (+0.4%).

```diff
diff --git a/physicsinformeddiffusionmodels_amd/csrc/k_attn_proj.hip b/physicsinformeddiffusionmodels_amd/csrc/k_attn_proj.hip
--- a/physicsinformeddiffusionmodels_amd/csrc/k_attn_proj.hip
+++ b/physicsinformeddiffusionmodels_amd/csrc/k_attn_proj.hip
@@ -1,4 +1,6 @@
 #include "pidm_launch.h"
+
+#include <type_traits>
 
 namespace pidm {
 
@@ -8,6 +10,14 @@
 
 __device__ __forceinline__ float lap_exp(float x) { return __expf(x); }
 __device__ __forceinline__ int lap_row(int r, int half) { return (r & 3) + 8 * (r >> 2) + 4 * half; }
+__device__ __forceinline__ int lap_min(int a, int b) { return a < b ? a : b; }
+
+__host__ __device__ constexpr int lap_six_a(int k) { return k == 0 ? 2 : (k == 2 || k == 3) ? 1 : 0; }
+__host__ __device__ constexpr int lap_six_b(int k) { return k == 1 ? 2 : (k == 2 || k == 4) ? 1 : 0; }
+static bool lap_pipe() {
+  const char* e = knob("PIDM_LAP_PIPE");
+  return !(e && !atoi(e));
+}
 
 static int lap_nper_div() {
   const char* e = knob("PIDM_LAP_NPER_DIV");
@@ -120,7 +130,7 @@
   while (g > 1 && ntiles % g) --g;
   return g < 1 ? 1 : g;
 }
-template <int CB>
+template <int CB, bool PIPE>
 __global__ void __launch_bounds__(512) lap_kctx_split_kernel(const float* __restrict__ xn, const float* __restrict__ wqkv,
                                                              float* __restrict__ part, int N, int heads, int nper) {
   constexpr int C = 32 * CB, RA = 6 * C + 16;
@@ -136,12 +146,24 @@
   const int b = blockIdx.x / NS, ns = blockIdx.x % NS;
   const int HD = heads * kLapDH;
   const float* xb = xn + ((size_t)b * N + (size_t)ns * nper) * C;
+  const int h = wave;
+  f32x4 wr[C / 16][2];
+  auto load_w = [&]() __attribute__((always_inline)) {
+    const float* wrow = wqkv + ((size_t)HD + h * kLapDH + l31) * C + 8 * half;
+#pragma unroll
+    for (int s = 0; s < C / 16; ++s) {
+      wr[s][0] = *reinterpret_cast<const f32x4*>(wrow + 16 * s);
+      wr[s][1] = *reinterpret_cast<const f32x4*>(wrow + 16 * s + 4);
+    }
+  };
+  if constexpr (PIPE)
+    if (h < heads) load_w();
   {
     constexpr int QN = C / 4, GP = 16 / QN;
     const int q = lane & (QN - 1), pb = (lane & 15) / QN, la = lane >> 4;
-    for (int sl = wave; sl < nper / (4 * GP); sl += 8) {
+    const int nsl = nper / (4 * GP);
+    auto stage = [&](const f32x4& v, int sl) __attribute__((always_inline)) {
       const int px = (sl * GP + pb) * 4 + la;
-      const f32x4 v = *reinterpret_cast<const f32x4*>(xb + (size_t)px * C + 4 * q);
       typedef unsigned u32x2_t __attribute__((ext_vector_type(2)));
       unsigned a0, a1, a2, b0, b1, b2;
       pidm_split3_pk(v[0], v[1], a0, a1, a2);
@@ -164,17 +186,30 @@
       *reinterpret_cast<u32x2_t*>(dt) = u32x2_t{a0, b0};
       *reinterpret_cast<u32x2_t*>(dt + (size_t)C * RT) = u32x2_t{a1, b1};
       *reinterpret_cast<u32x2_t*>(dt + (size_t)2 * C * RT) = u32x2_t{a2, b2};
+    };
+    auto quad = [&](int sl) __attribute__((always_inline)) {
+      return *reinterpret_cast<const f32x4*>(xb + (size_t)((sl * GP + pb) * 4 + la) * C + 4 * q);
+    };
+    if constexpr (!PIPE) {
+      for (int sl = wave; sl < nsl; sl += 8) stage(quad(sl), sl);
+    } else {
+      f32x4 v[4];
+#pragma unroll
+      for (int k = 0; k < 4; ++k) v[k] = quad(lap_min(wave + 8 * k, nsl - 1));
+      __builtin_amdgcn_sched_barrier(0);
+#pragma unroll
+      for (int k = 0; k < 4; ++k)
+        if (wave + 8 * k < nsl) stage(v[k], wave + 8 * k);
     }
   }
   __syncthreads();
-  const int h = wave;
   if (h >= heads) return;
   u32x4 wk[C / 16][3];
   {
-    const float* wrow = wqkv + ((size_t)HD + h * kLapDH + l31) * C + 8 * half;
+    if constexpr (!PIPE) load_w();
 #pragma unroll
     for (int s = 0; s < C / 16; ++s) {
-      const f32x4 w0 = *reinterpret_cast<const f32x4*>(wrow + 16 * s), w1 = *reinterpret_cast<const f32x4*>(wrow + 16 * s + 4);
+      const f32x4 w0 = wr[s][0], w1 = wr[s][1];
       unsigned p0[4], p1[4], p2[4];
       pidm_split3_pk(w0[0], w0[1], p0[0], p1[0], p2[0]);
       pidm_split3_pk(w0[2], w0[3], p0[1], p1[1], p2[1]);
@@ -198,68 +233,147 @@
   acc_ = pidm_mfma_bf16_32x32x16(a_[1], b_[0], acc_);                                                              \
   acc_ = pidm_mfma_bf16_32x32x16(a_[0], b_[1], acc_);                                                              \
   acc_ = pidm_mfma_bf16_32x32x16(a_[0], b_[0], acc_);
-  for (int t = 0; t < nper / 32; ++t) {
-    f32x16 kt;
-    for (int r = 0; r < 16; ++r) kt[r] = 0.f;
-    const char* arow = XA + (size_t)(t * 32 + l31) * RA + 16 * half;
-#pragma unroll
-    for (int s = 0; s < C / 16; ++s) {
-      u32x4 xa[3];
-#pragma unroll
-      for (int pc = 0; pc < 3; ++pc) xa[pc] = *reinterpret_cast<const u32x4*>(arow + pc * 2 * C + 32 * s);
-      PIDM_LAP_SIX(kt, xa, wk[s])
-    }
-    float tm = kt[0];
-#pragma unroll
-    for (int r = 1; r < 16; ++r) tm = fmaxf(tm, kt[r]);
-    tm = fmaxf(tm, pidm_other_half(tm));
-    if (__any(tm > mrun)) {
-      const float mn = fmaxf(mrun, tm);
-      const float f = lap_exp(mrun - mn);
-      zp *= f;
-      mrun = mn;
-      if (half == 0) fw[l31] = f;
-      PIDM_WAVE_LDS_SYNC();
-#pragma unroll
-      for (int q4 = 0; q4 < 4; ++q4) {
-        const f32x4 f4 = *reinterpret_cast<const f32x4*>(fw + 8 * q4 + 4 * half);
-#pragma unroll
-        for (int cb = 0; cb < CB; ++cb)
-#pragma unroll
-          for (int i = 0; i < 4; ++i) M[cb][4 * q4 + i] *= f4[i];
-      }
-      PIDM_WAVE_LDS_SYNC();
-    }
-#pragma unroll
-    for (int r = 0; r < 16; ++r) {
-      kt[r] = lap_exp(kt[r] - mrun);
-      zp += kt[r];
-    }
-#pragma unroll
-    for (int s = 0; s < 2; ++s) {
-      u32x4 ea[3];
-      {
-        unsigned p0[4], p1[4], p2[4];
-#pragma unroll
-        for (int j = 0; j < 4; ++j) pidm_split3_pk(kt[8 * s + 2 * j], kt[8 * s + 2 * j + 1], p0[j], p1[j], p2[j]);
-        ea[0] = u32x4{p0[0], p0[1], p0[2], p0[3]};
-        ea[1] = u32x4{p1[0], p1[1], p1[2], p1[3]};
-        ea[2] = u32x4{p2[0], p2[1], p2[2], p2[3]};
-      }
-#pragma unroll
-      for (int cb = 0; cb < CB; ++cb) {
-        u32x4 xb4[3];
-        const char* brow = XT + (size_t)(32 * cb + l31) * RT + (size_t)(t * 32 + 16 * s + 4 * half) * 2;
-#pragma unroll
-        for (int pc = 0; pc < 3; ++pc) {
-          typedef unsigned u32x2_t __attribute__((ext_vector_type(2)));
-          const u32x2_t lo = *reinterpret_cast<const u32x2_t*>(brow + (size_t)pc * C * RT);
-          const u32x2_t hi = *reinterpret_cast<const u32x2_t*>(brow + (size_t)pc * C * RT + 16);
-          xb4[pc] = u32x4{lo[0], lo[1], hi[0], hi[1]};
+  auto rescale = [&](float tm) __attribute__((always_inline)) {
+    const float mn = fmaxf(mrun, tm);
+    const float f = lap_exp(mrun - mn);
+    zp *= f;
+    mrun = mn;
+    if (half == 0) fw[l31] = f;
+    PIDM_WAVE_LDS_SYNC();
+#pragma unroll
+    for (int q4 = 0; q4 < 4; ++q4) {
+      const f32x4 f4 = *reinterpret_cast<const f32x4*>(fw + 8 * q4 + 4 * half);
+#pragma unroll
+      for (int cb = 0; cb < CB; ++cb)
+#pragma unroll
+        for (int i = 0; i < 4; ++i) M[cb][4 * q4 + i] *= f4[i];
+    }
+    PIDM_WAVE_LDS_SYNC();
+  };
+  auto bfrag = [&](u32x4 (&xb4)[3], int t, int s, int cb) __attribute__((always_inline)) {
+    const char* brow = XT + (size_t)(32 * cb + l31) * RT + (size_t)(t * 32 + 16 * s + 4 * half) * 2;
+#pragma unroll
+    for (int pc = 0; pc < 3; ++pc) {
+      typedef unsigned u32x2_t __attribute__((ext_vector_type(2)));
+      const u32x2_t lo = *reinterpret_cast<const u32x2_t*>(brow + (size_t)pc * C * RT);
+      const u32x2_t hi = *reinterpret_cast<const u32x2_t*>(brow + (size_t)pc * C * RT + 16);
+      xb4[pc] = u32x4{lo[0], lo[1], hi[0], hi[1]};
+    }
+  };
+  auto accum = [&](const u32x4 (&ea)[3], int t, int s) __attribute__((always_inline)) {
+#pragma unroll
+    for (int cb = 0; cb < CB; ++cb) {
+      u32x4 xb4[3];
+      bfrag(xb4, t, s, cb);
+      PIDM_LAP_SIX(M[cb], ea, xb4)
+    }
+  };
+  if constexpr (!PIPE) {
+    for (int t = 0; t < nper / 32; ++t) {
+      f32x16 kt;
+      for (int r = 0; r < 16; ++r) kt[r] = 0.f;
+      const char* arow = XA + (size_t)(t * 32 + l31) * RA + 16 * half;
+#pragma unroll
+      for (int s = 0; s < C / 16; ++s) {
+        u32x4 xa[3];
+#pragma unroll
+        for (int pc = 0; pc < 3; ++pc) xa[pc] = *reinterpret_cast<const u32x4*>(arow + pc * 2 * C + 32 * s);
+        PIDM_LAP_SIX(kt, xa, wk[s])
+      }
+      float tm = kt[0];
+#pragma unroll
+      for (int r = 1; r < 16; ++r) tm = fmaxf(tm, kt[r]);
+      tm = fmaxf(tm, pidm_other_half(tm));
+      if (__any(tm > mrun)) rescale(tm);
+#pragma unroll
+      for (int r = 0; r < 16; ++r) {
+        kt[r] = lap_exp(kt[r] - mrun);
+        zp += kt[r];
+      }
+#pragma unroll
+      for (int s = 0; s < 2; ++s) {
+        u32x4 ea[3];
+        {
+          unsigned p0[4], p1[4], p2[4];
+#pragma unroll
+          for (int j = 0; j < 4; ++j) pidm_split3_pk(kt[8 * s + 2 * j], kt[8 * s + 2 * j + 1], p0[j], p1[j], p2[j]);
+          ea[0] = u32x4{p0[0], p0[1], p0[2], p0[3]};
+          ea[1] = u32x4{p1[0], p1[1], p1[2], p1[3]};
+          ea[2] = u32x4{p2[0], p2[1], p2[2], p2[3]};
         }
-        PIDM_LAP_SIX(M[cb], ea, xb4)
-      }
-    }
+        accum(ea, t, s);
+      }
+    }
+  } else {
+    const int T = nper / 32;
+    constexpr int NM = 6 * (C / 16), NU = 24;
+    u32x4 xa[C / 16][3];
+    auto frags = [&](int t) __attribute__((always_inline)) {
+      const char* arow = XA + (size_t)(t * 32 + l31) * RA + 16 * half;
+#pragma unroll
+      for (int s = 0; s < C / 16; ++s)
+#pragma unroll
+        for (int pc = 0; pc < 3; ++pc) xa[s][pc] = *reinterpret_cast<const u32x4*>(arow + pc * 2 * C + 32 * s);
+    };
+    auto tile = [&](f32x16& kt, f32x16& kn, int t) __attribute__((always_inline)) {
+      const bool more = t + 1 < T;
+      frags(more ? t + 1 : t);
+      u32x4 bf[2][3];
+      if constexpr (CB == 1) {
+        bfrag(bf[0], t, 0, 0);
+        bfrag(bf[1], t, 1, 0);
+      }
+      __builtin_amdgcn_sched_barrier(0);
+      float tm = kt[0];
+#pragma unroll
+      for (int r = 1; r < 16; ++r) tm = fmaxf(tm, kt[r]);
+      tm = fmaxf(tm, pidm_other_half(tm));
+      if (__any(tm > mrun)) rescale(tm);
+      unsigned p[3][8];
+      auto vec = [&](auto NEXT_) __attribute__((always_inline)) {
+        constexpr bool NEXT = decltype(NEXT_)::value;
+        if constexpr (NEXT)
+          for (int r = 0; r < 16; ++r) kn[r] = 0.f;
+#pragma unroll
+        for (int i = 0; i < NM; ++i) {
+          if constexpr (NEXT) {
+            kn = pidm_mfma_bf16_32x32x16(xa[i / 6][lap_six_a(i % 6)], wk[i / 6][lap_six_b(i % 6)], kn);
+            __builtin_amdgcn_sched_barrier(0);
+          }
+#pragma unroll
+          for (int u = i * NU / NM; u < (i + 1) * NU / NM; ++u) {
+            if (u < 16) {
+              kt[u] = lap_exp(kt[u] - mrun);
+              zp += kt[u];
+            } else {
+              pidm_split3_pk(kt[2 * (u - 16)], kt[2 * (u - 16) + 1], p[0][u - 16], p[1][u - 16], p[2][u - 16]);
+            }
+          }
+          if constexpr (NEXT) __builtin_amdgcn_sched_barrier(0);
+        }
+      };
+      if (more) vec(std::true_type{});
+      else vec(std::false_type{});
+#pragma unroll
+      for (int s = 0; s < 2; ++s) {
+        const u32x4 ea[3] = {u32x4{p[0][4 * s], p[0][4 * s + 1], p[0][4 * s + 2], p[0][4 * s + 3]},
+                             u32x4{p[1][4 * s], p[1][4 * s + 1], p[1][4 * s + 2], p[1][4 * s + 3]},
+                             u32x4{p[2][4 * s], p[2][4 * s + 1], p[2][4 * s + 2], p[2][4 * s + 3]}};
+        if constexpr (CB == 1) { PIDM_LAP_SIX(M[0], ea, bf[s]) }
+        else accum(ea, t, s);
+      }
+    };
+    f32x16 k0, k1;
+    for (int r = 0; r < 16; ++r) k0[r] = 0.f;
+    frags(0);
+#pragma unroll
+    for (int s = 0; s < C / 16; ++s) { PIDM_LAP_SIX(k0, xa[s], wk[s]) }
+    int t = 0;
+    for (; t + 1 < T; t += 2) {
+      tile(k0, k1, t);
+      tile(k1, k0, t + 1);
+    }
+    if (t < T) tile(k0, k1, t);
   }
 #undef PIDM_LAP_SIX
   const float z = zp + pidm_other_half(zp);
@@ -420,6 +534,7 @@
   }
 }
 
+template <bool PIPE>
 __global__ void __launch_bounds__(512) lap_out_split_kernel(const float* __restrict__ xn, const float* __restrict__ wqkv,
                                                             const float* __restrict__ P, const float* __restrict__ bias,
                                                             const float* __restrict__ resid, float* __restrict__ y,
@@ -436,12 +551,23 @@
   const int wgs_per_img = (N / 32 + tiles_per_wg - 1) / tiles_per_wg;
   const int b = blockIdx.x / wgs_per_img, wg = blockIdx.x % wgs_per_img;
   typedef unsigned u32x2_t __attribute__((ext_vector_type(2)));
+  const int t_end = (wg + 1) * tiles_per_wg < N / 32 ? (wg + 1) * tiles_per_wg : N / 32;
+  const int tw = wg * tiles_per_wg + wave;
+  auto load_rows = [&](f32x4 (&xr)[C / 16][2], size_t pix) __attribute__((always_inline)) {
+#pragma unroll
+    for (int s = 0; s < C / 16; ++s) {
+      xr[s][0] = *reinterpret_cast<const f32x4*>(xn + pix * C + 16 * s + 8 * half);
+      xr[s][1] = *reinterpret_cast<const f32x4*>(xn + pix * C + 16 * s + 8 * half + 4);
+    }
+  };
+  f32x4 xr[C / 16][2];
+  if constexpr (PIPE)
+    if (tw < t_end) load_rows(xr, (size_t)b * N + (size_t)tw * 32 + l31);
   {
     const int q = lane & 7, pb = (lane >> 3) & 1, la = lane >> 4;
-    for (int sl = wave; sl < HD / 8; sl += 8) {
+    const int nsl = HD / 8;
+    auto stage = [&](const f32x4& v, const f32x4& w, int sl) __attribute__((always_inline)) {
       const int d = (sl * 2 + pb) * 4 + la;
-      const f32x4 v = *reinterpret_cast<const f32x4*>(wqkv + (size_t)d * C + 4 * q);
-      const f32x4 w = *reinterpret_cast<const f32x4*>(P + ((size_t)b * HD + d) * C + 4 * q);
       unsigned a0, a1, a2, b0, b1, b2;
       pidm_split3_pk(v[0], v[1], a0, a1, a2);
       pidm_split3_pk(v[2], v[3], b0, b1, b2);
@@ -463,6 +589,24 @@
       *reinterpret_cast<u32x2_t*>(dt) = u32x2_t{a0, b0};
       *reinterpret_cast<u32x2_t*>(dt + (size_t)C * RT) = u32x2_t{a1, b1};
       *reinterpret_cast<u32x2_t*>(dt + (size_t)2 * C * RT) = u32x2_t{a2, b2};
+    };
+    auto quad = [&](const float* src, int sl) __attribute__((always_inline)) {
+      return *reinterpret_cast<const f32x4*>(src + (size_t)((sl * 2 + pb) * 4 + la) * C + 4 * q);
+    };
+    const float* Pb = P + (size_t)b * HD * C;
+    if constexpr (!PIPE) {
+      for (int sl = wave; sl < nsl; sl += 8) stage(quad(wqkv, sl), quad(Pb, sl), sl);
+    } else {
+      f32x4 v[4], w[4];
+#pragma unroll
+      for (int k = 0; k < 4; ++k) {
+        v[k] = quad(wqkv, lap_min(wave + 8 * k, nsl - 1));
+        w[k] = quad(Pb, lap_min(wave + 8 * k, nsl - 1));
+      }
+      __builtin_amdgcn_sched_barrier(0);
+#pragma unroll
+      for (int k = 0; k < 4; ++k)
+        if (wave + 8 * k < nsl) stage(v[k], w[k], wave + 8 * k);
     }
   }
   __syncthreads();
@@ -473,71 +617,34 @@
   acc_ = pidm_mfma_bf16_32x32x16(a_[1], b_[0], acc_);                                                              \
   acc_ = pidm_mfma_bf16_32x32x16(a_[0], b_[1], acc_);                                                              \
   acc_ = pidm_mfma_bf16_32x32x16(a_[0], b_[0], acc_);
-  const int t_end = (wg + 1) * tiles_per_wg < N / 32 ? (wg + 1) * tiles_per_wg : N / 32;
-  for (int t = wg * tiles_per_wg + wave; t < t_end; t += 8) {
-    const size_t pix = (size_t)b * N + (size_t)t * 32 + l31;
-    u32x4 xb[C / 16][3];
+  auto split_rows = [&](u32x4 (&xb)[C / 16][3], const f32x4 (&xr)[C / 16][2]) __attribute__((always_inline)) {
 #pragma unroll
     for (int s = 0; s < C / 16; ++s) {
-      const f32x4 x0 = *reinterpret_cast<const f32x4*>(xn + pix * C + 16 * s + 8 * half);
-      const f32x4 x1 = *reinterpret_cast<const f32x4*>(xn + pix * C + 16 * s + 8 * half + 4);
       unsigned p0[4], p1[4], p2[4];
-      pidm_split3_pk(x0[0], x0[1], p0[0], p1[0], p2[0]);
-      pidm_split3_pk(x0[2], x0[3], p0[1], p1[1], p2[1]);
-      pidm_split3_pk(x1[0], x1[1], p0[2], p1[2], p2[2]);
-      pidm_split3_pk(x1[2], x1[3], p0[3], p1[3], p2[3]);
+      pidm_split3_pk(xr[s][0][0], xr[s][0][1], p0[0], p1[0], p2[0]);
+      pidm_split3_pk(xr[s][0][2], xr[s][0][3], p0[1], p1[1], p2[1]);
+      pidm_split3_pk(xr[s][1][0], xr[s][1][1], p0[2], p1[2], p2[2]);
+      pidm_split3_pk(xr[s][1][2], xr[s][1][3], p0[3], p1[3], p2[3]);
       xb[s][0] = u32x4{p0[0], p0[1], p0[2], p0[3]};
       xb[s][1] = u32x4{p1[0], p1[1], p1[2], p1[3]};
       xb[s][2] = u32x4{p2[0], p2[1], p2[2], p2[3]};
     }
-    f32x16 yacc;
-    for (int r = 0; r < 16; ++r) yacc[r] = 0.f;
-    for (int h = 0; h < heads; ++h) {
-      f32x16 qt;
-      for (int r = 0; r < 16; ++r) qt[r] = 0.f;
-      const char* wrow = WA + (size_t)(h * kLapDH + l31) * RA + 16 * half;
-#pragma unroll
-      for (int s = 0; s < C / 16; ++s) {
-        u32x4 wa[3];
-#pragma unroll
-        for (int pc = 0; pc < 3; ++pc) wa[pc] = *reinterpret_cast<const u32x4*>(wrow + pc * 2 * C + 32 * s);
-        PIDM_LAP_SIX(qt, wa, xb[s])
-      }
-      float mx = qt[0];
-#pragma unroll
-      for (int r = 1; r < 16; ++r) mx = fmaxf(mx, qt[r]);
-      mx = fmaxf(mx, pidm_other_half(mx));
-      float sm = 0.f;
-#pragma unroll
-      for (int r = 0; r < 16; ++r) {
-        qt[r] = lap_exp(qt[r] - mx);
-        sm += qt[r];
-      }
-      sm += pidm_other_half(sm);
-      const float inv = 1.f / sm;
-      if (half == 0) *reinterpret_cast<float2*>(qstat + (pix * heads + h) * 2) = make_float2(mx, inv);
-      const float sc = inv * scale;
-#pragma unroll
-      for (int s = 0; s < 2; ++s) {
-        u32x4 qb[3], pa[3];
-        {
-          unsigned p0[4], p1[4], p2[4];
-#pragma unroll
-          for (int j = 0; j < 4; ++j) pidm_split3_pk(qt[8 * s + 2 * j] * sc, qt[8 * s + 2 * j + 1] * sc, p0[j], p1[j], p2[j]);
-          qb[0] = u32x4{p0[0], p0[1], p0[2], p0[3]};
-          qb[1] = u32x4{p1[0], p1[1], p1[2], p1[3]};
-          qb[2] = u32x4{p2[0], p2[1], p2[2], p2[3]};
-        }
-        const char* prow = PT + (size_t)l31 * RT + (size_t)(h * kLapDH + 16 * s + 4 * half) * 2;
-#pragma unroll
-        for (int pc = 0; pc < 3; ++pc) {
-          const u32x2_t lo = *reinterpret_cast<const u32x2_t*>(prow + (size_t)pc * C * RT);
-          const u32x2_t hi = *reinterpret_cast<const u32x2_t*>(prow + (size_t)pc * C * RT + 16);
-          pa[pc] = u32x4{lo[0], lo[1], hi[0], hi[1]};
-        }
-        PIDM_LAP_SIX(yacc, pa, qb)
-      }
-    }
+  };
+  auto pfrag = [&](u32x4 (&pa)[3], int h, int s) __attribute__((always_inline)) {
+    const char* prow = PT + (size_t)l31 * RT + (size_t)(h * kLapDH + 16 * s + 4 * half) * 2;
+#pragma unroll
+    for (int pc = 0; pc < 3; ++pc) {
+      const u32x2_t lo = *reinterpret_cast<const u32x2_t*>(prow + (size_t)pc * C * RT);
+      const u32x2_t hi = *reinterpret_cast<const u32x2_t*>(prow + (size_t)pc * C * RT + 16);
+      pa[pc] = u32x4{lo[0], lo[1], hi[0], hi[1]};
+    }
+  };
+  auto accum = [&](f32x16& yacc, const u32x4 (&qb)[3], int h, int s) __attribute__((always_inline)) {
+    u32x4 pa[3];
+    pfrag(pa, h, s);
+    PIDM_LAP_SIX(yacc, pa, qb)
+  };
+  auto epilogue = [&](const f32x16& yacc, size_t pix) __attribute__((always_inline)) {
 #pragma unroll
     for (int q4 = 0; q4 < 4; ++q4) {
       const int c0 = 8 * q4 + 4 * half;
@@ -547,6 +654,141 @@
 #pragma unroll
       for (int i = 0; i < 4; ++i) o[i] = yacc[4 * q4 + i] + bv[i] + rv[i];
       *reinterpret_cast<f32x4*>(y + pix * C + c0) = o;
+    }
+  };
+  if constexpr (!PIPE) {
+    for (int t = wg * tiles_per_wg + wave; t < t_end; t += 8) {
+      const size_t pix = (size_t)b * N + (size_t)t * 32 + l31;
+      u32x4 xb[C / 16][3];
+      load_rows(xr, pix);
+      split_rows(xb, xr);
+      f32x16 yacc;
+      for (int r = 0; r < 16; ++r) yacc[r] = 0.f;
+      for (int h = 0; h < heads; ++h) {
+        f32x16 qt;
+        for (int r = 0; r < 16; ++r) qt[r] = 0.f;
+        const char* wrow = WA + (size_t)(h * kLapDH + l31) * RA + 16 * half;
+#pragma unroll
+        for (int s = 0; s < C / 16; ++s) {
+          u32x4 wa[3];
+#pragma unroll
+          for (int pc = 0; pc < 3; ++pc) wa[pc] = *reinterpret_cast<const u32x4*>(wrow + pc * 2 * C + 32 * s);
+          PIDM_LAP_SIX(qt, wa, xb[s])
+        }
+        float mx = qt[0];
+#pragma unroll
+        for (int r = 1; r < 16; ++r) mx = fmaxf(mx, qt[r]);
+        mx = fmaxf(mx, pidm_other_half(mx));
+        float sm = 0.f;
+#pragma unroll
+        for (int r = 0; r < 16; ++r) {
+          qt[r] = lap_exp(qt[r] - mx);
+          sm += qt[r];
+        }
+        sm += pidm_other_half(sm);
+        const float inv = 1.f / sm;
+        if (half == 0) *reinterpret_cast<float2*>(qstat + (pix * heads + h) * 2) = make_float2(mx, inv);
+        const float sc = inv * scale;
+#pragma unroll
+        for (int s = 0; s < 2; ++s) {
+          u32x4 qb[3];
+          {
+            unsigned p0[4], p1[4], p2[4];
+#pragma unroll
+            for (int j = 0; j < 4; ++j) pidm_split3_pk(qt[8 * s + 2 * j] * sc, qt[8 * s + 2 * j + 1] * sc, p0[j], p1[j], p2[j]);
+            qb[0] = u32x4{p0[0], p0[1], p0[2], p0[3]};
+            qb[1] = u32x4{p1[0], p1[1], p1[2], p1[3]};
+            qb[2] = u32x4{p2[0], p2[1], p2[2], p2[3]};
+          }
+          accum(yacc, qb, h, s);
+        }
+      }
+      epilogue(yacc, pix);
+    }
+  } else {
+    constexpr int NM = 6 * (C / 16), NU = 27;
+    u32x4 wa[C / 16][3];
+    auto frags = [&](int h) __attribute__((always_inline)) {
+      const char* wrow = WA + (size_t)(h * kLapDH + l31) * RA + 16 * half;
+#pragma unroll
+      for (int s = 0; s < C / 16; ++s)
+#pragma unroll
+        for (int pc = 0; pc < 3; ++pc) wa[s][pc] = *reinterpret_cast<const u32x4*>(wrow + pc * 2 * C + 32 * s);
+    };
+    for (int t = tw; t < t_end; t += 8) {
+      const size_t pix = (size_t)b * N + (size_t)t * 32 + l31;
+      u32x4 xb[C / 16][3];
+      split_rows(xb, xr);
+      __builtin_amdgcn_sched_barrier(0);
+      load_rows(xr, (size_t)b * N + (size_t)(t + 8 < t_end ? t + 8 : t) * 32 + l31);
+      __builtin_amdgcn_sched_barrier(0);
+      f32x16 yacc;
+      for (int r = 0; r < 16; ++r) yacc[r] = 0.f;
+      auto head = [&](f32x16& qt, f32x16& qn, int h) __attribute__((always_inline)) {
+        const bool more = h + 1 < heads;
+        frags(more ? h + 1 : h);
+        u32x4 pf[2][3];
+        pfrag(pf[0], h, 0);
+        pfrag(pf[1], h, 1);
+        __builtin_amdgcn_sched_barrier(0);
+        unsigned p[3][8];
+        float mx = qt[0], sm = 0.f, inv = 0.f, sc = 0.f;
+        auto vec = [&](auto NEXT_) __attribute__((always_inline)) {
+          constexpr bool NEXT = decltype(NEXT_)::value;
+          if constexpr (NEXT)
+            for (int r = 0; r < 16; ++r) qn[r] = 0.f;
+#pragma unroll
+          for (int i = 0; i < NM; ++i) {
+            if constexpr (NEXT) {
+              qn = pidm_mfma_bf16_32x32x16(wa[i / 6][lap_six_a(i % 6)], xb[i / 6][lap_six_b(i % 6)], qn);
+              __builtin_amdgcn_sched_barrier(0);
+            }
+#pragma unroll
+            for (int u = i * NU / NM; u < (i + 1) * NU / NM; ++u) {
+              if (u == 0) {
+#pragma unroll
+                for (int r = 1; r < 8; ++r) mx = fmaxf(mx, qt[r]);
+              } else if (u == 1) {
+#pragma unroll
+                for (int r = 8; r < 16; ++r) mx = fmaxf(mx, qt[r]);
+                mx = fmaxf(mx, pidm_other_half(mx));
+              } else if (u < 18) {
+                qt[u - 2] = lap_exp(qt[u - 2] - mx);
+                sm += qt[u - 2];
+              } else if (u == 18) {
+                sm += pidm_other_half(sm);
+                inv = 1.f / sm;
+                sc = inv * scale;
+              } else {
+                pidm_split3_pk(qt[2 * (u - 19)] * sc, qt[2 * (u - 19) + 1] * sc, p[0][u - 19], p[1][u - 19], p[2][u - 19]);
+              }
+            }
+            if constexpr (NEXT) __builtin_amdgcn_sched_barrier(0);
+          }
+        };
+        if (more) vec(std::true_type{});
+        else vec(std::false_type{});
+        if (half == 0) *reinterpret_cast<float2*>(qstat + (pix * heads + h) * 2) = make_float2(mx, inv);
+#pragma unroll
+        for (int s = 0; s < 2; ++s) {
+          const u32x4 qb[3] = {u32x4{p[0][4 * s], p[0][4 * s + 1], p[0][4 * s + 2], p[0][4 * s + 3]},
+                               u32x4{p[1][4 * s], p[1][4 * s + 1], p[1][4 * s + 2], p[1][4 * s + 3]},
+                               u32x4{p[2][4 * s], p[2][4 * s + 1], p[2][4 * s + 2], p[2][4 * s + 3]}};
+          PIDM_LAP_SIX(yacc, pf[s], qb)
+        }
+      };
+      f32x16 q0, q1;
+      for (int r = 0; r < 16; ++r) q0[r] = 0.f;
+      frags(0);
+#pragma unroll
+      for (int s = 0; s < C / 16; ++s) { PIDM_LAP_SIX(q0, wa[s], xb[s]) }
+      int h = 0;
+      for (; h + 1 < heads; h += 2) {
+        head(q0, q1, h);
+        head(q1, q0, h + 1);
+      }
+      if (h < heads) head(q0, q1, h);
+      epilogue(yacc, pix);
     }
   }
 #undef PIDM_LAP_SIX
@@ -609,7 +851,7 @@
     for (int r = 0; r < 16; ++r) o[(size_t)lap_row(r, half) * C + 32 * cb + l31] = G[cb][r];
 }
 
-template <int CB>
+template <int CB, bool PIPE>
 __global__ void __launch_bounds__(512) lap_g_split_kernel(const float* __restrict__ xn, const float* __restrict__ dy,
                                                           const float* __restrict__ wqkv, const float* __restrict__ qstat,
                                                           float* __restrict__ part, int N, int heads, int nper, float scale) {
@@ -619,19 +861,31 @@
   const int RT = nper * 2 + 16;
   char* XA = smem;
   char* YT = smem + (size_t)nper * RA;
+  float2* QS = reinterpret_cast<float2*>(YT + (size_t)3 * C * RT);
   const int tid = threadIdx.x, lane = tid & 63, half = lane >> 5, l31 = lane & 31;
   const int wave = __builtin_amdgcn_readfirstlane(tid >> 6);
   const int NS = N / nper;
   const int b = blockIdx.x / NS, ns = blockIdx.x % NS;
   const size_t pix0 = (size_t)b * N + (size_t)ns * nper;
+  const int h = wave;
+  f32x4 wr[C / 16][2];
+  auto load_w = [&]() __attribute__((always_inline)) {
+    const float* wrow = wqkv + ((size_t)h * kLapDH + l31) * C + 8 * half;
+#pragma unroll
+    for (int s = 0; s < C / 16; ++s) {
+      wr[s][0] = *reinterpret_cast<const f32x4*>(wrow + 16 * s);
+      wr[s][1] = *reinterpret_cast<const f32x4*>(wrow + 16 * s + 4);
+    }
+  };
+  if constexpr (PIPE)
+    if (h < heads) load_w();
   {
     constexpr int QN = C / 4, GP = 16 / QN;
     const int q = lane & (QN - 1), pb = (lane & 15) / QN, la = lane >> 4;
+    const int nsl = nper / (4 * GP);
     typedef unsigned u32x2_t __attribute__((ext_vector_type(2)));
-    for (int sl = wave; sl < nper / (4 * GP); sl += 8) {
+    auto stage = [&](const f32x4& v, const f32x4& w, int sl) __attribute__((always_inline)) {
       const int px = (sl * GP + pb) * 4 + la;
-      const f32x4 v = *reinterpret_cast<const f32x4*>(xn + (pix0 + px) * C + 4 * q);
-      const f32x4 w = *reinterpret_cast<const f32x4*>(dy + (pix0 + px) * C + 4 * q);
       unsigned a0, a1, a2, b0, b1, b2;
       pidm_split3_pk(v[0], v[1], a0, a1, a2);
       pidm_split3_pk(v[2], v[3], b0, b1, b2);
@@ -653,17 +907,40 @@
       *reinterpret_cast<u32x2_t*>(dt) = u32x2_t{a0, b0};
       *reinterpret_cast<u32x2_t*>(dt + (size_t)C * RT) = u32x2_t{a1, b1};
       *reinterpret_cast<u32x2_t*>(dt + (size_t)2 * C * RT) = u32x2_t{a2, b2};
+    };
+    auto quad = [&](const float* src, int sl) __attribute__((always_inline)) {
+      return *reinterpret_cast<const f32x4*>(src + (pix0 + (sl * GP + pb) * 4 + la) * C + 4 * q);
+    };
+    if constexpr (!PIPE) {
+      for (int sl = wave; sl < nsl; sl += 8) stage(quad(xn, sl), quad(dy, sl), sl);
+    } else {
+      f32x4 v[4], w[4];
+#pragma unroll
+      for (int k = 0; k < 4; ++k) {
+        v[k] = quad(xn, lap_min(wave + 8 * k, nsl - 1));
+        w[k] = quad(dy, lap_min(wave + 8 * k, nsl - 1));
+      }
+      const float2* qsrc = reinterpret_cast<const float2*>(qstat) + pix0 * heads;
+      float2 qv[4];
+#pragma unroll
+      for (int k = 0; k < 4; ++k) qv[k] = qsrc[lap_min(tid + 512 * k, nper * heads - 1)];
+      __builtin_amdgcn_sched_barrier(0);
+#pragma unroll
+      for (int k = 0; k < 4; ++k)
+        if (wave + 8 * k < nsl) stage(v[k], w[k], wave + 8 * k);
+#pragma unroll
+      for (int k = 0; k < 4; ++k)
+        if (tid + 512 * k < nper * heads) QS[tid + 512 * k] = qv[k];
     }
   }
   __syncthreads();
-  const int h = wave;
   if (h >= heads) return;
   u32x4 wq[C / 16][3];
   {
-    const float* wrow = wqkv + ((size_t)h * kLapDH + l31) * C + 8 * half;
+    if constexpr (!PIPE) load_w();
 #pragma unroll
     for (int s = 0; s < C / 16; ++s) {
-      const f32x4 w0 = *reinterpret_cast<const f32x4*>(wrow + 16 * s), w1 = *reinterpret_cast<const f32x4*>(wrow + 16 * s + 4);
+      const f32x4 w0 = wr[s][0], w1 = wr[s][1];
       unsigned p0[4], p1[4], p2[4];
       pidm_split3_pk(w0[0], w0[1], p0[0], p1[0], p2[0]);
       pidm_split3_pk(w0[2], w0[3], p0[1], p1[1], p2[1]);
@@ -685,48 +962,121 @@
   acc_ = pidm_mfma_bf16_32x32x16(a_[1], b_[0], acc_);                                                              \
   acc_ = pidm_mfma_bf16_32x32x16(a_[0], b_[1], acc_);                                                              \
   acc_ = pidm_mfma_bf16_32x32x16(a_[0], b_[0], acc_);
-  for (int t = 0; t < nper / 32; ++t) {
-    f32x16 qt;
-    for (int r = 0; r < 16; ++r) qt[r] = 0.f;
-    const char* arow = XA + (size_t)(t * 32 + l31) * RA + 16 * half;
-#pragma unroll
-    for (int s = 0; s < C / 16; ++s) {
-      u32x4 xa[3];
-#pragma unroll
-      for (int pc = 0; pc < 3; ++pc) xa[pc] = *reinterpret_cast<const u32x4*>(arow + pc * 2 * C + 32 * s);
-      PIDM_LAP_SIX(qt, xa, wq[s])
-    }
-    const float* st = qstat + ((pix0 + (size_t)t * 32) * heads + h) * 2;
-#pragma unroll
-    for (int r = 0; r < 16; ++r) {
-      const float2 s2 = *reinterpret_cast<const float2*>(st + (size_t)lap_row(r, half) * heads * 2);
-      qt[r] = lap_exp(qt[r] - s2.x) * s2.y * scale;
-    }
-#pragma unroll
-    for (int s = 0; s < 2; ++s) {
-      u32x4 ea[3];
-      {
-        unsigned p0[4], p1[4], p2[4];
-#pragma unroll
-        for (int j = 0; j < 4; ++j) pidm_split3_pk(qt[8 * s + 2 * j], qt[8 * s + 2 * j + 1], p0[j], p1[j], p2[j]);
-        ea[0] = u32x4{p0[0], p0[1], p0[2], p0[3]};
-        ea[1] = u32x4{p1[0], p1[1], p1[2], p1[3]};
-        ea[2] = u32x4{p2[0], p2[1], p2[2], p2[3]};
-      }
-#pragma unroll
-      for (int cb = 0; cb < CB; ++cb) {
-        u32x4 yb4[3];
-        const char* brow = YT + (size_t)(32 * cb + l31) * RT + (size_t)(t * 32 + 16 * s + 4 * half) * 2;
-#pragma unroll
-        for (int pc = 0; pc < 3; ++pc) {
-          typedef unsigned u32x2_t __attribute__((ext_vector_type(2)));
-          const u32x2_t lo = *reinterpret_cast<const u32x2_t*>(brow + (size_t)pc * C * RT);
-          const u32x2_t hi = *reinterpret_cast<const u32x2_t*>(brow + (size_t)pc * C * RT + 16);
-          yb4[pc] = u32x4{lo[0], lo[1], hi[0], hi[1]};
+  auto bfrag = [&](u32x4 (&yb4)[3], int t, int s, int cb) __attribute__((always_inline)) {
+    const char* brow = YT + (size_t)(32 * cb + l31) * RT + (size_t)(t * 32 + 16 * s + 4 * half) * 2;
+#pragma unroll
+    for (int pc = 0; pc < 3; ++pc) {
+      typedef unsigned u32x2_t __attribute__((ext_vector_type(2)));
+      const u32x2_t lo = *reinterpret_cast<const u32x2_t*>(brow + (size_t)pc * C * RT);
+      const u32x2_t hi = *reinterpret_cast<const u32x2_t*>(brow + (size_t)pc * C * RT + 16);
+      yb4[pc] = u32x4{lo[0], lo[1], hi[0], hi[1]};
+    }
+  };
+  auto accum = [&](const u32x4 (&ea)[3], int t, int s) __attribute__((always_inline)) {
+#pragma unroll
+    for (int cb = 0; cb < CB; ++cb) {
+      u32x4 yb4[3];
+      bfrag(yb4, t, s, cb);
+      PIDM_LAP_SIX(G[cb], ea, yb4)
+    }
+  };
+  if constexpr (!PIPE) {
+    for (int t = 0; t < nper / 32; ++t) {
+      f32x16 qt;
+      for (int r = 0; r < 16; ++r) qt[r] = 0.f;
+      const char* arow = XA + (size_t)(t * 32 + l31) * RA + 16 * half;
+#pragma unroll
+      for (int s = 0; s < C / 16; ++s) {
+        u32x4 xa[3];
+#pragma unroll
+        for (int pc = 0; pc < 3; ++pc) xa[pc] = *reinterpret_cast<const u32x4*>(arow + pc * 2 * C + 32 * s);
+        PIDM_LAP_SIX(qt, xa, wq[s])
+      }
+      const float* st = qstat + ((pix0 + (size_t)t * 32) * heads + h) * 2;
+#pragma unroll
+      for (int r = 0; r < 16; ++r) {
+        const float2 s2 = *reinterpret_cast<const float2*>(st + (size_t)lap_row(r, half) * heads * 2);
+        qt[r] = lap_exp(qt[r] - s2.x) * s2.y * scale;
+      }
+#pragma unroll
+      for (int s = 0; s < 2; ++s) {
+        u32x4 ea[3];
+        {
+          unsigned p0[4], p1[4], p2[4];
+#pragma unroll
+          for (int j = 0; j < 4; ++j) pidm_split3_pk(qt[8 * s + 2 * j], qt[8 * s + 2 * j + 1], p0[j], p1[j], p2[j]);
+          ea[0] = u32x4{p0[0], p0[1], p0[2], p0[3]};
+          ea[1] = u32x4{p1[0], p1[1], p1[2], p1[3]};
+          ea[2] = u32x4{p2[0], p2[1], p2[2], p2[3]};
         }
-        PIDM_LAP_SIX(G[cb], ea, yb4)
-      }
-    }
+        accum(ea, t, s);
+      }
+    }
+  } else {
+    const int T = nper / 32;
+    constexpr int NM = 6 * (C / 16), NU = 24;
+    u32x4 xa[C / 16][3];
+    auto frags = [&](int t) __attribute__((always_inline)) {
+      const char* arow = XA + (size_t)(t * 32 + l31) * RA + 16 * half;
+#pragma unroll
+      for (int s = 0; s < C / 16; ++s)
+#pragma unroll
+        for (int pc = 0; pc < 3; ++pc) xa[s][pc] = *reinterpret_cast<const u32x4*>(arow + pc * 2 * C + 32 * s);
+    };
+    auto tile = [&](f32x16& qt, f32x16& qn, int t) __attribute__((always_inline)) {
+      const bool more = t + 1 < T;
+      float2 s2[16];
+      const float2* st = QS + (size_t)t * 32 * heads + h;
+#pragma unroll
+      for (int r = 0; r < 16; ++r) s2[r] = st[(size_t)lap_row(r, half) * heads];
+      frags(more ? t + 1 : t);
+      u32x4 bf[2][3];
+      if constexpr (CB == 1) {
+        bfrag(bf[0], t, 0, 0);
+        bfrag(bf[1], t, 1, 0);
+      }
+      __builtin_amdgcn_sched_barrier(0);
+      unsigned p[3][8];
+      auto vec = [&](auto NEXT_) __attribute__((always_inline)) {
+        constexpr bool NEXT = decltype(NEXT_)::value;
+        if constexpr (NEXT)
+          for (int r = 0; r < 16; ++r) qn[r] = 0.f;
+#pragma unroll
+        for (int i = 0; i < NM; ++i) {
+          if constexpr (NEXT) {
+            qn = pidm_mfma_bf16_32x32x16(xa[i / 6][lap_six_a(i % 6)], wq[i / 6][lap_six_b(i % 6)], qn);
+            __builtin_amdgcn_sched_barrier(0);
+          }
+#pragma unroll
+          for (int u = i * NU / NM; u < (i + 1) * NU / NM; ++u) {
+            if (u < 16) qt[u] = lap_exp(qt[u] - s2[u].x) * s2[u].y * scale;
+            else pidm_split3_pk(qt[2 * (u - 16)], qt[2 * (u - 16) + 1], p[0][u - 16], p[1][u - 16], p[2][u - 16]);
+          }
+          if constexpr (NEXT) __builtin_amdgcn_sched_barrier(0);
+        }
+      };
+      if (more) vec(std::true_type{});
+      else vec(std::false_type{});
+#pragma unroll
+      for (int s = 0; s < 2; ++s) {
+        const u32x4 ea[3] = {u32x4{p[0][4 * s], p[0][4 * s + 1], p[0][4 * s + 2], p[0][4 * s + 3]},
+                             u32x4{p[1][4 * s], p[1][4 * s + 1], p[1][4 * s + 2], p[1][4 * s + 3]},
+                             u32x4{p[2][4 * s], p[2][4 * s + 1], p[2][4 * s + 2], p[2][4 * s + 3]}};
+        if constexpr (CB == 1) { PIDM_LAP_SIX(G[0], ea, bf[s]) }
+        else accum(ea, t, s);
+      }
+    };
+    f32x16 q0, q1;
+    for (int r = 0; r < 16; ++r) q0[r] = 0.f;
+    frags(0);
+#pragma unroll
+    for (int s = 0; s < C / 16; ++s) { PIDM_LAP_SIX(q0, xa[s], wq[s]) }
+    int t = 0;
+    for (; t + 1 < T; t += 2) {
+      tile(q0, q1, t);
+      tile(q1, q0, t + 1);
+    }
+    if (t < T) tile(q0, q1, t);
   }
 #undef PIDM_LAP_SIX
   float* o = part + ((size_t)blockIdx.x * heads + h) * (size_t)(32 * C);
@@ -1263,6 +1613,7 @@
   constexpr int C = 32 * CB;
   const char* spe = knob("PIDM_LAP_SPLIT");
   const bool split1 = !(spe && !atoi(spe));
+  const bool pipe = lap_pipe();
   const int nper = split1 ? lap_nper_split(N, C) : lap_nper(N, C, 1), NS = N / nper;
   float* kst = saved;
   float* Mmat = kst + (size_t)B * heads * 64;
@@ -1280,11 +1631,13 @@
     const size_t ldss = (size_t)nper * (6 * C + 16) + (size_t)3 * C * (nper * 2 + 16) + 8 * 32 * sizeof(float);
     static bool attr_s = false;
     if (!attr_s) {
-      (void)hipFuncSetAttribute(reinterpret_cast<const void*>(&lap_kctx_split_kernel<CB>), hipFuncAttributeMaxDynamicSharedMemorySize, 160 * 1024 - 256);
+      (void)hipFuncSetAttribute(reinterpret_cast<const void*>(&lap_kctx_split_kernel<CB, false>), hipFuncAttributeMaxDynamicSharedMemorySize, 160 * 1024 - 256);
+      (void)hipFuncSetAttribute(reinterpret_cast<const void*>(&lap_kctx_split_kernel<CB, true>), hipFuncAttributeMaxDynamicSharedMemorySize, 160 * 1024 - 256);
       attr_s = true;
     }
     PIDM_PROF_NAME("lap_kctx_split_kernel");
-    hipLaunchKernelGGL(HIP_KERNEL_NAME(lap_kctx_split_kernel<CB>), dim3(B * NS), dim3(512), ldss, st, xn, wqkv, scratch, N, heads, nper);
+    if (pipe) hipLaunchKernelGGL(HIP_KERNEL_NAME(lap_kctx_split_kernel<CB, true>), dim3(B * NS), dim3(512), ldss, st, xn, wqkv, scratch, N, heads, nper);
+    else hipLaunchKernelGGL(HIP_KERNEL_NAME(lap_kctx_split_kernel<CB, false>), dim3(B * NS), dim3(512), ldss, st, xn, wqkv, scratch, N, heads, nper);
   } else {
     hipLaunchKernelGGL(HIP_KERNEL_NAME(lap_kctx_kernel<CB>), dim3(B * NS), dim3(512), lds1, st, xn, wqkv, scratch, N, heads, nper);
   }
@@ -1304,11 +1657,13 @@
     const size_t ldso = (size_t)HD * (6 * C + 16) + (size_t)3 * C * (HD * 2 + 16);
     static bool attr_o = false;
     if (!attr_o) {
-      (void)hipFuncSetAttribute(reinterpret_cast<const void*>(&lap_out_split_kernel), hipFuncAttributeMaxDynamicSharedMemorySize, 160 * 1024 - 256);
+      (void)hipFuncSetAttribute(reinterpret_cast<const void*>(&lap_out_split_kernel<false>), hipFuncAttributeMaxDynamicSharedMemorySize, 160 * 1024 - 256);
+      (void)hipFuncSetAttribute(reinterpret_cast<const void*>(&lap_out_split_kernel<true>), hipFuncAttributeMaxDynamicSharedMemorySize, 160 * 1024 - 256);
       attr_o = true;
     }
     PIDM_PROF_NAME("lap_out_split_kernel");
-    hipLaunchKernelGGL(lap_out_split_kernel, dim3(wg8), dim3(512), ldso, st, xn, wqkv, P, bias, resid, y, qstat, N, heads, tp8, 0.17677669529663687f);
+    if (pipe) hipLaunchKernelGGL(lap_out_split_kernel<true>, dim3(wg8), dim3(512), ldso, st, xn, wqkv, P, bias, resid, y, qstat, N, heads, tp8, 0.17677669529663687f);
+    else hipLaunchKernelGGL(lap_out_split_kernel<false>, dim3(wg8), dim3(512), ldso, st, xn, wqkv, P, bias, resid, y, qstat, N, heads, tp8, 0.17677669529663687f);
   } else {
     hipLaunchKernelGGL(HIP_KERNEL_NAME(lap_out_kernel<CB>), dim3(wgs), dim3(256), lds3, st, xn, wqkv, P, bias, resid, y, qstat, N, heads, tpw,
                        0.17677669529663687f);
@@ -1349,13 +1704,18 @@
   const char* spe = knob("PIDM_LAP_SPLIT");
   if (!(spe && !atoi(spe))) {
     const size_t ldss = (size_t)np2 * (6 * C + 16) + (size_t)3 * C * (np2 * 2 + 16);
+    const size_t ldsq = (size_t)np2 * heads * sizeof(float2);
     static bool attr_s = false;
     if (!attr_s) {
-      (void)hipFuncSetAttribute(reinterpret_cast<const void*>(&lap_g_split_kernel<CB>), hipFuncAttributeMaxDynamicSharedMemorySize, 160 * 1024 - 256);
+      (void)hipFuncSetAttribute(reinterpret_cast<const void*>(&lap_g_split_kernel<CB, false>), hipFuncAttributeMaxDynamicSharedMemorySize, 160 * 1024 - 256);
+      (void)hipFuncSetAttribute(reinterpret_cast<const void*>(&lap_g_split_kernel<CB, true>), hipFuncAttributeMaxDynamicSharedMemorySize, 160 * 1024 - 256);
       attr_s = true;
     }
     PIDM_PROF_NAME("lap_g_split_kernel");
-    hipLaunchKernelGGL(HIP_KERNEL_NAME(lap_g_split_kernel<CB>), dim3(B * NS2), dim3(512), ldss, st, xn, dy, wqkv, qstat, scratch, N, heads, np2, scale);
+    if (lap_pipe())
+      hipLaunchKernelGGL(HIP_KERNEL_NAME(lap_g_split_kernel<CB, true>), dim3(B * NS2), dim3(512), ldss + ldsq, st, xn, dy, wqkv, qstat, scratch, N, heads, np2, scale);
+    else
+      hipLaunchKernelGGL(HIP_KERNEL_NAME(lap_g_split_kernel<CB, false>), dim3(B * NS2), dim3(512), ldss, st, xn, dy, wqkv, qstat, scratch, N, heads, np2, scale);
   } else {
     hipLaunchKernelGGL(HIP_KERNEL_NAME(lap_g_kernel<CB>), dim3(B * NS2), dim3(512), lds1, st, xn, dy, wqkv, qstat, scratch, N, heads, np2, scale);
   }
```
